# tqch/v-diffusion-torch

Measured on AMD Instinct MI355X. Metric: train_images_per_sec, higher is better.
Workload: dtype fp32 (bf16x3 split products in the tile-engine GEMMs)

## Files before the change

include/vdiff_hip.h:

```cpp
#ifndef VDIFF_HIP_H
#define VDIFF_HIP_H
#include <stddef.h>
#include <stdint.h>

#ifdef __cplusplus
extern "C" {
#endif

#define VD_VERSION 100

int         vd_version(void);
const char* vd_last_error(void);

int         vd_set_reserved_cus(int32_t n);
int         vd_reserved_cus(void);

int         vd_mfma_calibrate(float* sink, unsigned long long* stamps, int32_t blocks, int32_t iters, uint32_t seed, void* stream);

enum { VD_ROW = 0,
       VD_COL = 1,
       VD_IM2COL = 2 };

typedef struct vd_gemm_desc {
    const float* A; const float* B; float* C;
// ... 34 lines not shown
int vd_conv3x3_wino_supported(int32_t nimg, int32_t H, int32_t W, int32_t Cin, int32_t Cout, int64_t ldx, int64_t ldy, int64_t ldres);
int vd_conv3x3_wino(const float* xin, int64_t ldx, const float* U, const float* bias, const float* res, int64_t ldres,
                    float* y, int64_t ldy, int32_t nimg, int32_t H, int32_t W, int32_t Cin, int32_t Cout,
                    float* stats_part, void* stream);
int vd_conv3x3_wgrad_wino_supported(int32_t nimg, int32_t H, int32_t W, int32_t Cin, int32_t Cout, int64_t ldx, int64_t lddy);
size_t vd_conv3x3_wgrad_wino_ws_bytes(int32_t nimg, int32_t H, int32_t W, int32_t Cin, int32_t Cout);
int vd_conv3x3_wgrad_wino(const float* xin, int64_t ldx, const float* dy, int64_t lddy, int32_t nimg, int32_t H, int32_t W,
                          int32_t Cin, int32_t Cout, float* dw_oihw, float* dbias, int32_t Cin_w, int32_t Cout_w,
                          int32_t accumulate, float* ws, size_t ws_bytes, void* stream);
int vd_conv3x3_wgrad_wino_phase(const float* xin, int64_t ldx, const float* dy, int64_t lddy, int32_t nimg, int32_t H, int32_t W,
                                int32_t Cin, int32_t Cout, float* dw_oihw, float* dbias, int32_t Cin_w, int32_t Cout_w,
                                int32_t accumulate, float* ws, size_t ws_bytes, int32_t phase, void* stream);
int vd_wino_last_kernel(void);
int vd_wino_wgrad_last_kernel(void);
#ifdef VD_PROBES
int vd_wino_set_probe(unsigned long long* buf);
int vd_wino43_set_probe(unsigned long long* buf);
int vd_gn_set_spin_probe(unsigned* buf);
#endif
int vd_wino_pack(const float* w_oihw, int32_t Cout, int32_t Cin, float* uf , float* ud , void* stream);
int vd_conv3x3_dgrad_wino43_supported(int32_t nimg, int32_t H, int32_t W, int32_t Cin, int32_t Cout, int64_t lddy, int64_t lddx);
size_t vd_wino43_u_floats(int32_t Cout, int32_t Cin);
int vd_conv3x3_dgrad_wino43(const float* dy, int64_t lddy, const float* U43, float* dx, int64_t lddx, int32_t nimg, int32_t H, int32_t W,
                            int32_t Cin, int32_t Cout, void* stream);
int vd_wino43_last_kernel(void);
int vd_wino43_pack(const float* w_oihw, int32_t Cout, int32_t Cin, float* U43, void* stream);
int vd_wino43_pack_batched(const int64_t* items_dev, int32_t n, int64_t total_blocks, void* stream);
int vd_conv3x3_wino43_preferred(int32_t nimg, int32_t H, int32_t W, int32_t N);
int vd_conv3x3_wino43_fwd_supported(int32_t nimg, int32_t H, int32_t W, int32_t Cin, int32_t Cout, int64_t ldx, int64_t ldy, int64_t ldres);
int vd_wino43_pack_fwd(const float* w_oihw, int32_t Cout, int32_t Cin, float* U43f, void* stream);
int vd_conv3x3_wino43_fwd_chunk_rows(int32_t H, int32_t W);
int vd_conv3x3_wino43_fwd(const float* xin, int64_t ldx, const float* U43f, const float* bias, const float* res, int64_t ldres, float* y,
                          int64_t ldy, int32_t nimg, int32_t H, int32_t W, int32_t Cin, int32_t Cout, float* stats_part, void* stream);
int vd_conv3x3_wgrad_wino43_supported(int32_t nimg, int32_t H, int32_t W, int32_t Cin, int32_t Cout, int64_t ldx, int64_t lddy);
size_t vd_conv3x3_wgrad_wino43_ws_bytes(int32_t nimg, int32_t H, int32_t W, int32_t Cin, int32_t Cout);
int vd_conv3x3_wgrad_wino43(const float* xin, int64_t ldx, const float* dy, int64_t lddy, int32_t nimg, int32_t H, int32_t W,
                            int32_t Cin, int32_t Cout, float* dw_oihw, float* dbias, int32_t Cin_w, int32_t Cout_w,
                            int32_t accumulate, float* ws, size_t ws_bytes, void* stream);
int vd_conv3x3_wgrad_wino43_phase(const float* xin, int64_t ldx, const float* dy, int64_t lddy, int32_t nimg, int32_t H, int32_t W,
                                  int32_t Cin, int32_t Cout, float* dw_oihw, float* dbias, int32_t Cin_w, int32_t Cout_w,
                                  int32_t accumulate, float* ws, size_t ws_bytes, int32_t phase, void* stream);
int vd_wino43_wgrad_last_kernel(void);

int vd_wino_pack_batched(const int64_t* items_dev, int32_t n, int64_t total_blocks, void* stream);

int vd_im2col3x3(const float* x, int64_t ldx, float* xc , int32_t nimg, int32_t H, int32_t W, int32_t C, void* stream);
int vd_tap_gather(const float* z, int64_t ldz, const float* bias, float* out, int64_t ldo, int32_t nimg, int32_t H, int32_t W, int32_t Cout, void* stream);
int vd_tap_spread(const float* dy, int64_t lddy, float* dz, int64_t ldz, int32_t nimg, int32_t H, int32_t W, int32_t Cout, void* stream);
int vd_thin_wgrad_finish(const float* g, int32_t Cout_w, int32_t Cin, int32_t Cin_w, float* dw_oihw, int32_t accumulate,
                         const float* colsum, int32_t cs_stride, int32_t cs_off, float* dbias, void* stream);

size_t vd_conv3x3_wgrad_ws_bytes(int32_t nimg, int32_t H, int32_t W, int32_t Cin, int32_t Cout);
int vd_conv3x3_wgrad(const float* xin, int64_t ldx, const float* dy, int64_t lddy,
                     int32_t nimg, int32_t H, int32_t W, int32_t Cin, int32_t Cout,
                     float* dw_oihw, float* dbias, int32_t Cin_w, int32_t Cout_w, int32_t accumulate,
                     float* ws, size_t ws_bytes, void* stream);
int vd_conv3x3_wgrad_phase(const float* xin, int64_t ldx, const float* dy, int64_t lddy,
                           int32_t nimg, int32_t H, int32_t W, int32_t Cin, int32_t Cout,
                           float* dw_oihw, float* dbias, int32_t Cin_w, int32_t Cout_w, int32_t accumulate,
                           float* ws, size_t ws_bytes, int32_t phase, void* stream);

int vd_pack_conv3x3(const float* w_oihw, int32_t Cout_w, int32_t Cin_w,
                    float* wf, int32_t Cin_p, float* wd, int32_t Cout_p, void* stream);
int vd_pack_conv3x3_batched(const int64_t* items_dev, int32_t n, int64_t total_blocks, void* stream);

enum { VD_RS_NONE = 0, VD_RS_DOWN = 1, VD_RS_UP = 2 };

size_t vd_gn_ws_bytes(int32_t nimg, int32_t HW, int32_t C);
int vd_gn_stats(const float* x, int64_t ldx, int32_t nimg, int32_t HW, int32_t C, int32_t G, float eps,
                float* stats, float* ws, size_t ws_bytes, void* stream);

int vd_gn_stats_from_partials(const float* part1, int32_t C1, int32_t chunks1, const float* part2, int32_t C2, int32_t chunks2,
                              int32_t nimg, int32_t HW, int32_t G, float eps, float* stats, void* stream);

int vd_gn_coef_from_partials(const float* part1, int32_t C1, int32_t chunks1, const float* part2, int32_t C2, int32_t chunks2,
                             int32_t nimg, int32_t HW, int32_t G, float eps, const float* gamma, const float* beta,
                             const float* film, float* coef, void* stream);

int vd_gn_apply(const float* x, int64_t ldx, const float* stats, const float* gamma, const float* beta,
                const float* film, int32_t act, float p_drop, uint64_t seed,
                int32_t resample, float* y, int64_t ldy,
                int32_t nimg, int32_t H, int32_t W, int32_t C, int32_t G, float* coef, void* stream);

int vd_gn_apply_from_partials(const float* x, int64_t ldx, const float* part1, int32_t C1, int32_t chunks1, const float* part2, int32_t C2,
                              int32_t chunks2, const float* gamma, const float* beta, const float* film, int32_t act, float p_drop,
                              uint64_t seed, int32_t resample, float* y, int64_t ldy, int32_t nimg, int32_t H, int32_t W, int32_t C,
                              int32_t G, float eps, float* coef, void* stream);

int vd_gn_apply_bwd(const float* dy, int64_t lddy, const float* x, int64_t ldx, const float* coef,
                    const float* gamma, const float* beta, const float* film, int32_t act, float p_drop, uint64_t seed,
                    int32_t resample, const float* add, int64_t ldadd, float* dx, int64_t lddx, int32_t accumulate_dx,
                    float* dfilm, float* dgamma, float* dbeta, int32_t accumulate_params,
                    int32_t nimg, int32_t H, int32_t W, int32_t C, int32_t G,
                    float* ws, size_t ws_bytes, void* stream);
int vd_gn_bwd_last_kernel(void);
int vd_gn_apply_bwd_keep(const float* dy, int64_t lddy, const float* x, int64_t ldx, const float* coef, const float* gamma,
                         const float* beta, const float* film, int32_t act, float p_drop, uint64_t seed, int32_t resample,
                         const float* add, int64_t ldadd, float* dx, int64_t lddx, int32_t accumulate_dx, float* dfilm, float* pgb_keep,
                         int32_t nimg, int32_t H, int32_t W, int32_t C, int32_t G, float* ws, size_t ws_bytes, void* stream);
int vd_gn_param_sums_batched(const int64_t* items_dev, int32_t n, int64_t total_blocks, void* stream);

size_t vd_colsum_ws_bytes(int64_t M, int32_t N);
int vd_colsum(const float* x, int64_t ldx, int64_t M, int32_t N, float* out, int32_t accumulate,
              float* ws, size_t ws_bytes, void* stream);
int vd_axpby(const float* x, int64_t ldx, float alpha, float* y, int64_t ldy, float beta, int64_t rows, int32_t C, void* stream);
int vd_silu(const float* x, float* y, int64_t n, void* stream);
int vd_silu_bwd(const float* x, const float* dy, float* dx, int64_t n, int32_t accumulate, void* stream);
int vd_softmax_rows(float* s, int64_t rows, int32_t L, void* stream);
int vd_softmax_rows_bwd(const float* p, float* dp, int64_t rows, int32_t L, float alpha, void* stream);

int vd_attn_supported(int32_t L, int32_t hd, int32_t backward);
int vd_attn_fwd(const float* q, const float* k, const float* v, int64_t ld, float* o, int64_t ldo, float* lse, int32_t B,
                int32_t nh, int32_t L, int32_t hd, float scale, void* stream);
int vd_attn_bwd(const float* q, const float* k, const float* v, int64_t ld, const float* o, int64_t ldo, const float* dout,
                int64_t lddo, const float* lse, float* delta, float* dq, float* dk, float* dv, int64_t ldd, int32_t B,
                int32_t nh, int32_t L, int32_t hd, float scale, void* stream);
int vd_attn_bwd_phase(const float* q, const float* k, const float* v, int64_t ld, const float* o, int64_t ldo, const float* dout,
                      int64_t lddo, const float* lse, float* delta, float* dq, float* dk, float* dv, int64_t ldd, int32_t B,
                      int32_t nh, int32_t L, int32_t hd, float scale, int32_t phase, void* stream);

int vd_nchw_to_nhwc(const float* x, float* y, int32_t nimg, int32_t C, int32_t H, int32_t W, int64_t ldy, void* stream);
// ... 55 lines not shown
```

v-diffusion-torch_amd/csrc/common.h:

```cpp
#pragma once
#include <hip/hip_runtime.h>
#include <stdint.h>
#include <stdio.h>
#include "../../include/vdiff_hip.h"

typedef float f32x4 __attribute__((ext_vector_type(4)));
typedef float f32x16 __attribute__((ext_vector_type(16)));

typedef float f32x2 __attribute__((ext_vector_type(2)));

#ifdef VD_PROBES
constexpr bool VD_PROBE_BUILD = true;
#else
constexpr bool VD_PROBE_BUILD = false;
#endif

void vd_set_error(const char* fmt, ...);
int vd_cu_count(void);
int vd_persistent_cus(void);
int vd_gemm_grouped_wgrad_kblk(const float* const* A, const float* const* B, float* const* C, float* const* colsum, int32_t count, int32_t M,
                               int32_t N, int32_t K, int64_t lda, int64_t ldb, int64_t ldc, int32_t splitk, float* ws, size_t ws_bytes,
                               void* stream, int64_t a_kblk, int64_t b_kblk, int32_t slabs_only);
int vd_gemm_grouped_wgrad_used_slabs(int32_t count, int32_t M, int32_t N, int32_t K, int32_t splitk);
extern thread_local int vd_g_last_tile;
inline int vd_tile_code(bool tr, bool spl, int kt, int bm, int bn) {
    return ((((tr ? 1 : 0) + (spl ? 2 : 0)) * 100 + kt) * 1000 + bm) * 1000 + bn;
}

#define VD_REQUIRE(cond, ...)                                   \
    do { if (!(cond)) { vd_set_error(__VA_ARGS__); return 1; } } while (0)

#define VD_LAUNCH_CHECK(name)                                                            \
    do { hipError_t e_ = hipGetLastError();                                              \
         if (e_ != hipSuccess) { vd_set_error("%s: %s", name, hipGetErrorString(e_)); return 2; } } while (0)

static inline bool vd_aligned16(const void* p) { return (reinterpret_cast<uintptr_t>(p) & 15) == 0; }

__device__ __forceinline__ float vd_sigmoid(float x) { return __builtin_amdgcn_rcpf(1.0f + __expf(-x)); }

__device__ __forceinline__ void vd_philox4(uint64_t seed, uint64_t ctr, uint32_t out[4]) {
    uint32_t k0 = (uint32_t)seed, k1 = (uint32_t)(seed >> 32);
    uint32_t c0 = (uint32_t)ctr, c1 = (uint32_t)(ctr >> 32), c2 = 0x243F6A88u, c3 = 0x85A308D3u;
#pragma unroll
    for (int r = 0; r < 10; ++r) {
        uint64_t p0 = (uint64_t)0xD2511F53u * c0, p1 = (uint64_t)0xCD9E8D57u * c2;
        uint32_t n0 = (uint32_t)(p1 >> 32) ^ c1 ^ k0, n2 = (uint32_t)(p0 >> 32) ^ c3 ^ k1;
        c1 = (uint32_t)p1; c3 = (uint32_t)p0; c0 = n0; c2 = n2;
        k0 += 0x9E3779B9u; k1 += 0xBB67AE85u;
    }
    out[0] = c0; out[1] = c1; out[2] = c2; out[3] = c3;
}
__device__ __forceinline__ f32x4 vd_dropout_scale4(uint64_t seed, uint64_t vec_index, float p) {
    uint32_t r[4];
    vd_philox4(seed, vec_index, r);
    const float inv = 1.0f / (1.0f - p);
    f32x4 m;
#pragma unroll
    for (int j = 0; j < 4; ++j) m[j] = ((r[j] >> 8) * (1.0f / 16777216.0f) >= p) ? inv : 0.0f;
    return m;
}
```

v-diffusion-torch_amd/csrc/gemm.hip:

```cpp
#include "common.h"
#include <math.h>
#include <stdlib.h>
#include <type_traits>

namespace {

constexpr int KT = 32;
#ifndef VD_GEMM_SPLIT_DEFAULT
#define VD_GEMM_SPLIT_DEFAULT 1
#endif

struct GemmArgs {
    const float* A; const float* B; float* C; const float* bias; const float* R;
    int M, N, K;
    long long lda, ldb, ldc, ldr;
    int nh;
    long long sAb, sAh, sBb, sBh, sCb, sCh, sRb, sRh;
    float alpha; int accumulate;
    int H, W, Cin;
    int kt_total, kt_per_split;
    long long slab_stride;
    float* colsum; int colsum_accumulate;
    int probe;
    float* stats; int stats_hw;
    long long sBias;
    int group_S;
    int lgW, lgHW;
    long long a_kblk, b_kblk;
};

__device__ __forceinline__ int PB(const GemmArgs& p) { return VD_PROBE_BUILD ? p.probe : 0; }

__device__ __forceinline__ int row_swz(int row, int chunk) { return row * KT + ((chunk ^ ((row >> 1) & 7)) << 2); }

template <int BM, int BN, int AK, int BK, bool SPLITK>
__global__ __launch_bounds__(256, 2) void gemm_kernel(const GemmArgs p) {
    __shared__ __attribute__((aligned(16))) float smem[2 * (BM + BN) * KT];
    float* As = smem;
    float* Bs = smem + 2 * BM * KT;

    constexpr int MT = BM / 64, NT = BN / 64;
    constexpr int AIT = BM / 32, BIT = BN / 32;
    constexpr int A_CPR = BM / 4, A_RPP = 256 / A_CPR;
    constexpr int B_CPR = BN / 4, B_RPP = 256 / B_CPR;

    const int tid = threadIdx.x, lane = tid & 63, wave = tid >> 6;
    const int li = lane & 31, lh = lane >> 5;
    const int wm = (wave >> 1) * (BM / 2), wn = (wave & 1) * (BN / 2);
    const int m0 = blockIdx.y * BM;
    int n0 = blockIdx.x * BN;
    int tapN = 0, ci0 = 0;
    if (BK == VD_IM2COL) {
        const int cchN = (p.Cin + BN - 1) / BN;
        tapN = blockIdx.x / cchN;
        ci0 = (blockIdx.x % cchN) * BN;
        n0 = tapN * p.Cin + ci0;
    }
    const float* A = p.A;
    const float* B = p.B;
    float* C = p.C;
    const float* R = p.R;
// ... 378 lines not shown
            const int rowoff = (GROUPED && p.a_kblk) ? (kk >> 4) * (int)p.a_kblk + (kk & 15) * (int)p.lda : kk * (int)p.lda;
            voA[j] = (m0 + cm < p.M) ? (unsigned)(rowoff + cm) * 4u : OOB;
            kcA[j] = kk; mkA[j] = 0;
        } else {
            const int row = q * RRPP + lane / RLPR;
            const int c = (lane % RLPR) ^ swz_of<KT>(row);
            const int m = m0 + row;
            kcA[j] = c * 4;
            voA[j] = (m < p.M) ? (unsigned)(row * (int)p.lda + c * 4) * 4u : OOB;
            unsigned mk = 0;
            if (AK == VD_IM2COL) {
                int y, x;
                pix_yx(p, m, y, x);
                const unsigned xm = (x > 0 ? 1u : 0u) | 2u | (x < p.W - 1 ? 4u : 0u);
                mk = (y > 0 ? xm : 0u) | (xm << 3) | (y < p.H - 1 ? xm << 6 : 0u);
            }
            mkA[j] = mk;
        }
    }
#pragma unroll
    for (int j = 0; j < BIT; ++j) {
        const int q = j * 4 + wave;
        if (BK == VD_ROW) {
            const int row = q * RRPP + lane / RLPR;
            const int c = (lane % RLPR) ^ swz_of<KT>(row);
            kcB[j] = c * 4;
            voB[j] = (n0 + row < p.N) ? (unsigned)(row * (int)p.ldb + c * 4) * 4u : OOB;
            by[j] = bx[j] = 0;
        } else {
            const int kk = q * B_RPP + lane / B_LPR, cn = (lane % B_LPR) * 4;
            kcB[j] = kk;
            const bool ok = (BK == VD_IM2COL) ? (ci0 + cn < p.Cin) : (n0 + cn < p.N);
            const int rowoff = (GROUPED && BK == VD_COL && p.b_kblk) ? (kk >> 4) * (int)p.b_kblk + (kk & 15) * (int)p.ldb : kk * (int)p.ldb;
            voB[j] = ok ? (unsigned)(rowoff + cn) * 4u : OOB;
            if (BK == VD_IM2COL) pix_yx(p, kt_begin * KT + kk, by[j], bx[j]);
            else by[j] = bx[j] = 0;
        }
    }
    const float* Ablk = (AK == VD_COL) ? A + m0 : A + (long long)m0 * p.lda;
    const float* Bblk = (BK == VD_ROW) ? B + (long long)n0 * p.ldb : ((BK == VD_COL) ? B + n0 : B + ci0);
    const long long tapoffB = (BK == VD_IM2COL) ? (long long)((tapN / 3 - 1) * p.W + (tapN % 3 - 1)) * p.ldb : 0;

#ifndef VD_ISSUE_IN
#define VD_ISSUE_IN 2
#endif
    constexpr bool ISSUE_IN = VD_ISSUE_IN == 2 ? (AK == VD_COL) : (VD_ISSUE_IN == 1);
    struct Prep { const float* pA; const float* pB; unsigned vA[AIT], vB[BIT]; };
    auto prep_tiles = [&](int kt, Prep& P) {
        {
            const int tap = tapA, c0 = ccA * KT;
            long long aoff;
            int kwidth;
            if (AK == VD_IM2COL) { aoff = (long long)((tap / 3 - 1) * p.W + (tap % 3 - 1)) * p.lda + c0; kwidth = p.Cin - c0; }
            else if (AK == VD_ROW) { aoff = (long long)kt * KT; kwidth = p.K - kt * KT; }
            else { aoff = (GROUPED && p.a_kblk) ? (long long)kt * (KT / 16) * p.a_kblk : (long long)kt * KT * p.lda; kwidth = p.K - kt * KT; }
            P.pA = Ablk + aoff;
#pragma unroll
            for (int j = 0; j < AIT; ++j) {
                unsigned vo = voA[j];
                if (kcA[j] >= kwidth) vo = OOB;
                if (AK == VD_IM2COL && !((mkA[j] >> tap) & 1u)) vo = OOB;
                P.vA[j] = vo;
            }
        }
        {
            long long boff;
            int kwidth;
            if (BK == VD_ROW) {
                if (AK == VD_IM2COL) { boff = (long long)tapA * p.Cin + ccA * KT; kwidth = p.Cin - ccA * KT; }
                else { boff = (long long)kt * KT; kwidth = p.K - kt * KT; }
            } else { boff = ((GROUPED && BK == VD_COL && p.b_kblk) ? (long long)kt * (KT / 16) * p.b_kblk : (long long)kt * KT * p.ldb) + tapoffB; kwidth = p.K - kt * KT; }
            P.pB = Bblk + boff;
            const int dy = tapN / 3 - 1, dx = tapN % 3 - 1;
// ... 399 lines not shown
            if (lh == 0 && mrow < p.M) {
                const int chunks = p.stats_hw / (BM / 2);
                float* o = p.stats + ((long long)(mrow / p.stats_hw) * chunks + (mrow % p.stats_hw) / (BM / 2)) * 2 * p.N + n;
                o[0] = st1; o[p.N] = st2;
            }
        }
    }
    stamp_end();
}

template <int BM, int BN, int AK, int BK, bool SPLITK, int KT, bool TR, bool GROUPED = false>
__global__ __launch_bounds__(256, (KT == 16 ? VD_KT16_BLOCKS : 2)) void gemm_dma_kernel(const GemmArgs p,
                                                                                          const std::conditional_t<GROUPED, GroupPtrs, NoGroup> gp) {
    gemm_dma_body<BM, BN, AK, BK, SPLITK, KT, TR, GROUPED, false>(p, gp);
}
template <int BM, int BN, int AK, int BK, bool SPLITK, int KT, bool TR, bool GROUPED = false>
__global__ __launch_bounds__(256, (KT == 16 ? VD_SPL_BLOCKS : 2)) void gemm_split_kernel(const GemmArgs p,
                                                                                           const std::conditional_t<GROUPED, GroupPtrs, NoGroup> gp) {
    gemm_dma_body<BM, BN, AK, BK, SPLITK, KT, TR, GROUPED, true>(p, gp);
}

__global__ __launch_bounds__(512) void wgrad_planes256_kernel(const GemmArgs p, const GroupPtrs gp) {
    constexpr int BM = 256, BN = 256, KTT = 16, NBUF = 3, STG = (BM + BN) * KTT;
    __shared__ __attribute__((aligned(1024))) float smem[NBUF * STG];
    typedef float f32x2 __attribute__((ext_vector_type(2)));
    const int tid = threadIdx.x, lane = tid & 63;
    const int wave = __builtin_amdgcn_readfirstlane(tid >> 6);
    const int li = lane & 31, lh = lane >> 5;
    const int wm = (wave >> 1) * 64, wn = (wave & 1) * 128;
    const int tbx = blockIdx.x, tby = blockIdx.y, tbz = blockIdx.z;
    const int m0 = tby * BM, n0 = tbx * BN;
    const int e = tbz / p.group_S, slab = tbz - e * p.group_S;
    const float* A = gp.A[e] + m0;
    const float* B = gp.B[e] + n0;
    const int kt_begin = slab * p.kt_per_split, kt_end = min(kt_begin + p.kt_per_split, p.kt_total);
    float* C = p.C + (long long)tbz * p.slab_stride;

    auto issue = [&](int kt, int buf) {
        float* as = smem + buf * STG;
        float* bs = as + BM * KTT;
        const int rec = kt < kt_end ? (int)OOB : 0;
        const __amdgpu_buffer_rsrc_t rsA = make_rsrc(A + (p.a_kblk ? (long long)kt * p.a_kblk : (long long)kt * KTT * p.lda), rec);
        const __amdgpu_buffer_rsrc_t rsB = make_rsrc(B + (p.b_kblk ? (long long)kt * p.b_kblk : (long long)kt * KTT * p.ldb), rec);
#pragma unroll
        for (int h = 0; h < 2; ++h) {
            const int kk = wave + 8 * h;
            __builtin_amdgcn_raw_ptr_buffer_load_lds(rsA, (lds_ptr_t)(as + kk * BM), 16, lane * 16, kk * (int)p.lda * 4, 0, 0);
            __builtin_amdgcn_raw_ptr_buffer_load_lds(rsB, (lds_ptr_t)(bs + kk * BN), 16, lane * 16, kk * (int)p.ldb * 4, 0, 0);
        }
    };

    f32x16 acc[2][4];
#pragma unroll
    for (int a = 0; a < 2; ++a)
#pragma unroll
        for (int b = 0; b < 4; ++b)
#pragma unroll
            for (int r = 0; r < 16; ++r) acc[a][b][r] = 0.f;
    float csum[2] = {0.f, 0.f};
    const bool do_cs = p.colsum != nullptr && tbx == 0 && (wave & 1) == 0;

    if (kt_begin < kt_end) {
        issue(kt_begin, 0);
        issue(kt_begin + 1, 1);
        asm volatile("s_waitcnt vmcnt(4)" ::: "memory");
        asm volatile("s_waitcnt lgkmcnt(0)\n\ts_barrier" ::: "memory");
        int buf = 0;
        for (int kt = kt_begin; kt < kt_end; ++kt) {
            const float* as = smem + buf * STG;
            const float* bs = as + BM * KTT;
            issue(kt + 2, buf >= 1 ? buf - 1 : 2);
            float fa[2][8];
            f32x4 fbq[8];
#pragma unroll
            for (int j = 0; j < 8; ++j) {
                const f32x2 v = *reinterpret_cast<const f32x2*>(as + (8 * lh + j) * BM + wm + 2 * li);
                fa[0][j] = v[0]; fa[1][j] = v[1];
                fbq[j] = *reinterpret_cast<const f32x4*>(bs + (8 * lh + j) * BN + wn + 4 * li);
            }
            bf16x8 ah[2], am[2], al[2];
#pragma unroll
// ... 400 lines not shown
    return g;
}
}

extern "C" int vd_gemm_grouped_wgrad_auto_split(int32_t count, int32_t M, int32_t N, int32_t K, int32_t min_slabs, int32_t max_slabs) {
    const int tile = choose_tile(M, N, false, (long long)count * 8, 0);
    const bool p256 = planes256(count, M, N, K);
    long long nm, nn;
    grouped_tiles(tile, p256, M, N, &nm, &nn);
    const long long blocks = nm * nn * count;
    const long long slots = (long long)vd_cu_count() * (p256 ? 1 : (tile == 0 && blocks * (min_slabs > 1 ? min_slabs : 1) >= GROUPED_K16_MIN_WGS / 2 ? 4 : TILES[tile].per_cu));
    int lo = min_slabs > 1 ? min_slabs : 1, hi = max_slabs > lo ? max_slabs : lo;
    const int kmax = K / 256 > 1 ? K / 256 : 1;
    if (hi > kmax) hi = kmax;
    if (lo > hi) lo = hi;
    int best = lo;
    double best_eff = -1.0;
    for (int s = lo; s <= hi; ++s) {
        const long long wgs = blocks * s, rounds = (wgs + slots - 1) / slots;
        double eff = (double)wgs / (double)(rounds * slots);
        eff *= 1.0 - 0.004 * s;
        if (eff > best_eff) { best_eff = eff; best = s; }
    }
    return best;
}

extern "C" size_t vd_gemm_grouped_wgrad_ws_bytes(int32_t count, int32_t M, int32_t N, int32_t splitk) {
    return (size_t)count * (splitk > 1 ? splitk : 1) * ((size_t)M * N + M) * sizeof(float);
}

extern "C" int vd_gemm_grouped_wgrad(const float* const* A, const float* const* B, float* const* C, float* const* colsum, int32_t count,
                                     int32_t M, int32_t N, int32_t K, int64_t lda, int64_t ldb, int64_t ldc, int32_t splitk, float* ws,
                                     size_t ws_bytes, void* stream) {
    return vd_gemm_grouped_wgrad_kblk(A, B, C, colsum, count, M, N, K, lda, ldb, ldc, splitk, ws, ws_bytes, stream, 0, 0, 0);
}

int vd_gemm_grouped_wgrad_used_slabs(int32_t count, int32_t M, int32_t N, int32_t K, int32_t splitk) {
    return plan_grouped(count, M, N, K, splitk > 1 ? splitk : 1).used;
}

int vd_gemm_grouped_wgrad_kblk(const float* const* A, const float* const* B, float* const* C, float* const* colsum, int32_t count,
                               int32_t M, int32_t N, int32_t K, int64_t lda, int64_t ldb, int64_t ldc, int32_t splitk, float* ws,
                               size_t ws_bytes, void* stream, int64_t a_kblk, int64_t b_kblk, int32_t slabs_only) {
    VD_REQUIRE(A && B && C && count > 0 && count <= VD_GROUP_MAX, "vd_gemm_grouped_wgrad: 1..%d entries (got %d)", VD_GROUP_MAX, count);
    VD_REQUIRE(M > 0 && N > 0 && K > 0 && M % 4 == 0 && N % 4 == 0 && lda % 4 == 0 && ldb % 4 == 0 && ldc >= N,
               "vd_gemm_grouped_wgrad: M, N, lda, ldb must be multiples of 4 (M=%d N=%d)", M, N);
    const int S = splitk > 1 ? splitk : 1;
    VD_REQUIRE(ws && ws_bytes >= vd_gemm_grouped_wgrad_ws_bytes(count, M, N, S), "vd_gemm_grouped_wgrad: workspace too small");
    GemmArgs a = {};
    GroupPtrs gp = {};
    GroupOut go = {};
    for (int e = 0; e < count; ++e) {
        VD_REQUIRE(A[e] && B[e] && C[e] && vd_aligned16(A[e]) && vd_aligned16(B[e]), "vd_gemm_grouped_wgrad: entry %d: null / unaligned operand", e);
        gp.A[e] = A[e]; gp.B[e] = B[e]; go.C[e] = C[e]; go.cs[e] = colsum ? colsum[e] : nullptr;
    }
    a.A = A[0]; a.B = B[0];
    a.M = M; a.N = N; a.K = K; a.lda = lda; a.ldb = ldb; a.ldc = N; a.ldr = 0; a.nh = 1;
    a.alpha = 1.f; a.lgW = a.lgHW = -1; a.probe = 0;
    a.a_kblk = a_kblk; a.b_kblk = b_kblk;
    VD_REQUIRE(a_kblk >= 0 && b_kblk >= 0 && a_kblk % 4 == 0 && b_kblk % 4 == 0 && 2 * a_kblk + 16 * lda + 128 < 0x70000000LL / 4 &&
               2 * b_kblk + 16 * ldb + 128 < 0x70000000LL / 4, "vd_gemm_grouped_wgrad: K-block strides outside the LDS-DMA kernel's range");
    VD_REQUIRE(dma_in_range(a), "vd_gemm_grouped_wgrad: operands outside the LDS-DMA kernel's range (alignment / row pitch)");
    const GroupedPlan g = plan_grouped(count, M, N, K, S);
    const int used = g.used;
    a.kt_total = g.kt_total; a.kt_per_split = g.kt_per_split; a.group_S = used;
    a.slab_stride = (long long)M * N;
    a.C = ws;
    float* cpart = ws + (long long)count * used * a.slab_stride;
    a.colsum = colsum ? cpart : nullptr;
    const dim3 grid((unsigned)g.nn, (unsigned)g.nm, (unsigned)(count * used));
    hipStream_t st = (hipStream_t)stream;
    if (g.p256) {
        vd_g_last_tile = vd_tile_code(true, true, 16, 256, 256);
        hipLaunchKernelGGL(wgrad_planes256_kernel, grid, dim3(512), 0, st, a, gp);
    } else if (g.tile == 0 && g.k16) launch_grouped<128, 128, 16>(a, gp, grid, st);
    else if (g.tile == 0) launch_grouped<128, 128>(a, gp, grid, st);
    else if (g.tile == 1) launch_grouped<128, 64>(a, gp, grid, st);
    else if (g.tile == 2) launch_grouped<64, 128>(a, gp, grid, st);
    else launch_grouped<64, 64>(a, gp, grid, st);
    VD_LAUNCH_CHECK("gemm_dma_kernel(grouped)");
    if (slabs_only) return 0;
    const long long tot = (long long)M * N;
    hipLaunchKernelGGL(reduce_slabs_grouped_kernel, dim3((unsigned)((tot + 255) / 256), (unsigned)count), dim3(256), 0, st, ws, used,
                       a.slab_stride, M, N, go, (long long)ldc, cpart);
    VD_LAUNCH_CHECK("reduce_slabs_grouped_kernel");
    return 0;
}

thread_local int vd_g_last_tile = 0;
extern "C" int vd_gemm_last_tile(void) { return vd_g_last_tile; }

extern "C" int vd_gemm(const vd_gemm_desc* d, void* stream) {
// ... 127 lines not shown
```

v-diffusion-torch_amd/csrc/norm.hip:

```cpp
#include "common.h"
#include <stdlib.h>

namespace {

constexpr int PPC = 128;

template <bool NT>
__device__ __forceinline__ f32x4 ld_stream(const float* p) {
    if (NT) return __builtin_nontemporal_load(reinterpret_cast<const f32x4*>(p));
    return *reinterpret_cast<const f32x4*>(p);
}
template <bool NT>
__device__ __forceinline__ void st_stream(float* p, f32x4 v) {
    if (NT) __builtin_nontemporal_store(v, reinterpret_cast<f32x4*>(p));
    else *reinterpret_cast<f32x4*>(p) = v;
}

struct ReduceArgs {
    const float* x; long long ldx;
    const float* dy; long long lddy;
    const float* coef;
    int act; float p_drop; unsigned long long seed; int resample; int has_norm;
    int H, W;
    long long HW;
// ... 279 lines not shown
    const float* ximg = p.x + (long long)b * p.H * p.W * p.ldx;
    float* yimg = p.y + (long long)b * Ho * Wo * p.ldy;
    if (p.resample == VD_RS_NONE) {
        for (int i = r; i < np; i += 4 * rows) {
            f32x4 v[4];
#pragma unroll
            for (int u = 0; u < 4; ++u)
                if (i + u * rows < np) v[u] = *reinterpret_cast<const f32x4*>(ximg + (long long)(p0 + i + u * rows) * p.ldx + c4);
#pragma unroll
            for (int u = 0; u < 4; ++u)
                if (i + u * rows < np) {
                    const int po = p0 + i + u * rows;
                    *reinterpret_cast<f32x4*>(yimg + (long long)po * p.ldy + c4) = fwd_val(p, v[u], po, c4, sc, of, b);
                }
        }
        return;
    }
    for (int i = r; i < np; i += rows) {
        const int po = p0 + i;
        f32x4 out;
        {
            const int yo = po / Wo, xo = po - yo * Wo;
            if (p.resample == VD_RS_UP) out = fwd_one(p, ximg, (yo >> 1) * p.W + (xo >> 1), c4, sc, of, b);
            else {
                const int q = (2 * yo) * p.W + 2 * xo;
                out = (fwd_one(p, ximg, q, c4, sc, of, b) + fwd_one(p, ximg, q + 1, c4, sc, of, b) +
                       fwd_one(p, ximg, q + p.W, c4, sc, of, b) + fwd_one(p, ximg, q + p.W + 1, c4, sc, of, b)) * 0.25f;
            }
        }
        *reinterpret_cast<f32x4*>(yimg + (long long)po * p.ldy + c4) = out;
    }
}

__global__ __launch_bounds__(256) void gn_bwd_finalize_kernel(const float* part, int chunks, const float* coef,
                                                              const float* gamma, const float* beta, const float* film,
                                                              int C, int G, long long HW, float* q, float* dfilm,
                                                              float* pgb) {
    extern __shared__ float sh[];
    float* k1 = sh; float* k2 = sh + C; float* gm = sh + 2 * C;
    const int b = blockIdx.x, cg = C / G;
    const float* cf = coef + (long long)b * 4 * C;
    for (int c = threadIdx.x; c < C; c += blockDim.x) {
        float s1 = 0.f, s2 = 0.f;
        for (int ch = 0; ch < chunks; ++ch) {
            const float* pp = part + ((long long)(b * chunks + ch) * 2) * C;
            s1 += pp[c]; s2 += pp[C + c];
        }
        float fs = 1.f;
        if (film) {
            fs = 1.f + film[(long long)b * 2 * C + C + c];
            dfilm[(long long)b * 2 * C + c] = s1;
            dfilm[(long long)b * 2 * C + C + c] = gamma[c] * s2 + beta[c] * s1;
        }
        const float k = gamma[c] * fs;
        k1[c] = k * s1; k2[c] = k * s2;
        pgb[((long long)b * 2) * C + c] = fs * s2;
        pgb[((long long)b * 2 + 1) * C + c] = fs * s1;
    }
    __syncthreads();
    if (threadIdx.x < G) {
        float m1 = 0.f, m2 = 0.f;
        for (int c = threadIdx.x * cg; c < (threadIdx.x + 1) * cg; ++c) { m1 += k1[c]; m2 += k2[c]; }
        const float inv = 1.f / ((float)cg * (float)HW);
        gm[threadIdx.x] = m1 * inv; gm[G + threadIdx.x] = m2 * inv;
    }
    __syncthreads();
// ... 442 lines not shown
    const long long Wo = resample == VD_RS_DOWN ? W / 2 : (resample == VD_RS_UP ? W * 2 : W);
    const int Cba = pick_cb(C);
    VD_REQUIRE(C % Cba == 0 && Cba % 4 == 0 && Cba <= 1024 && nimg <= 65535, "vd_gn_apply: cannot split C=%d / nimg=%d", C, nimg);
    hipLaunchKernelGGL(gn_apply_kernel<false>, dim3((unsigned)((Ho * Wo + APIX - 1) / APIX), nimg, C / Cba), dim3(256), 0, st, p, Cba, PartArgs{});
    VD_LAUNCH_CHECK("gn_apply_kernel");
    return 0;
}

extern "C" int vd_gn_apply_from_partials(const float* x, int64_t ldx, const float* part1, int32_t C1, int32_t chunks1, const float* part2,
                                         int32_t C2, int32_t chunks2, const float* gamma, const float* beta, const float* film, int32_t act,
                                         float p_drop, uint64_t seed, int32_t resample, float* y, int64_t ldy, int32_t nimg, int32_t H,
                                         int32_t W, int32_t C, int32_t G, float eps, float* coef, void* stream) {
    hipStream_t st = (hipStream_t)stream;
    VD_REQUIRE(x && y && part1 && gamma && beta, "vd_gn_apply_from_partials: null operand");
    VD_REQUIRE(C % 4 == 0 && ldx % 4 == 0 && ldy % 4 == 0 && C % G == 0 && C1 + C2 == C && C1 > 0 && chunks1 > 0,
               "vd_gn_apply_from_partials: bad channel split C=%d C1=%d C2=%d G=%d", C, C1, C2, G);
    VD_REQUIRE(C2 == 0 || (part2 && chunks2 > 0), "vd_gn_apply_from_partials: second source incomplete");
    VD_REQUIRE(resample != VD_RS_DOWN || (H % 2 == 0 && W % 2 == 0), "vd_gn_apply_from_partials: odd size cannot be average-pooled");
    VD_REQUIRE(vd_aligned16(x) && vd_aligned16(y) && (!coef || vd_aligned16(coef)), "vd_gn_apply_from_partials: operands must be 16-byte aligned");
    ApplyArgs p = {x, ldx, coef, 1, act, p_drop, seed, resample, y, ldy, nimg, H, W, C};
    PartArgs q = {part1, C1, chunks1, part2, C2, chunks2, G, eps, gamma, beta, film, coef};
    const long long Ho = resample == VD_RS_DOWN ? H / 2 : (resample == VD_RS_UP ? H * 2 : H);
    const long long Wo = resample == VD_RS_DOWN ? W / 2 : (resample == VD_RS_UP ? W * 2 : W);
    const int cg = C / G;
    int Cba = pick_cb(C);
    if (Cba % cg) {
        Cba = 0;
        for (int k = G; k >= 1; --k) if (G % k == 0 && (k * cg) % 4 == 0 && k * cg <= 1024) { Cba = k * cg; break; }
    }
    VD_REQUIRE(Cba > 0 && C % Cba == 0 && Cba % 4 == 0 && Cba % cg == 0 && Cba <= 1024 && Cba / cg <= 256 && nimg <= 65535,
               "vd_gn_apply_from_partials: cannot split C=%d into whole-group channel ranges", C);
    hipLaunchKernelGGL(gn_apply_kernel<true>, dim3((unsigned)((Ho * Wo + APIX - 1) / APIX), nimg, C / Cba), dim3(256), 0, st, p, Cba, q);
    VD_LAUNCH_CHECK("gn_apply_kernel<from partials>");
    return 0;
}

static int gn_apply_bwd_impl(const float* dy, int64_t lddy, const float* x, int64_t ldx, const float* coef,
                             const float* gamma, const float* beta, const float* film, int32_t act, float p_drop,
                             uint64_t seed, int32_t resample, const float* add, int64_t ldadd, float* dx, int64_t lddx,
                             int32_t accumulate_dx, float* dfilm, float* dgamma, float* dbeta, int32_t accumulate_params,
                             int32_t nimg, int32_t H, int32_t W, int32_t C, int32_t G, float* ws, size_t ws_bytes,
                             float* pgb_keep, void* stream) {
    hipStream_t st = (hipStream_t)stream;
    VD_REQUIRE(C % 4 == 0 && lddy % 4 == 0 && lddx % 4 == 0, "vd_gn_apply_bwd: C/ld must be multiples of 4");
    const int has_norm = gamma != nullptr;
    const long long HW = (long long)H * W;
    BwdApplyArgs a = {};
    ReduceArgs& p = a.r;
    p.x = x; p.ldx = ldx; p.dy = dy; p.lddy = lddy; p.coef = coef; p.act = act; p.p_drop = p_drop; p.seed = seed;
    p.resample = resample; p.has_norm = has_norm; p.H = H; p.W = W; p.HW = HW; p.C = C; p.nimg = nimg;
    p.chunks = (int)((HW + PPC - 1) / PPC);
    a.add = add; a.ldadd = ldadd; a.dx = dx; a.lddx = lddx; a.accumulate_dx = accumulate_dx;
    g_last_gn_bwd = has_norm ? -1 : 0;
    if (has_norm) {
        VD_REQUIRE(x && coef && beta && ((dgamma && dbeta) || pgb_keep) && C % G == 0 && ldx % 4 == 0, "vd_gn_apply_bwd: missing norm operands");
        VD_REQUIRE(!film || dfilm, "vd_gn_apply_bwd: film given without dfilm");
        VD_REQUIRE(ws && ws_bytes >= vd_gn_ws_bytes(nimg, (int)HW, C), "vd_gn_apply_bwd: workspace too small");
        const int Cb = pick_cb(C);
        VD_REQUIRE(C % Cb == 0 && Cb % 4 == 0 && Cb <= 1024, "vd_gn_apply_bwd: cannot split C=%d", C);
        float* part = ws;
        float* q = part + (long long)nimg * p.chunks * 2 * C;
        float* pgb = pgb_keep ? pgb_keep : q + (long long)nimg * 3 * C;
        p.part = part;
        static const bool two_pass = getenv("VD_GN_TWO_PASS") != nullptr;
        int CS = fused_slab(C, G);
        static const bool wide = !(getenv("VD_GN_WIDE") && atoi(getenv("VD_GN_WIDE")) == 0);
// ... 125 lines not shown
```

v-diffusion-torch_amd/csrc/wino43.hip:

```cpp
#include "common.h"
#include <type_traits>

namespace {

typedef __attribute__((address_space(3))) void* lds_ptr_t;
constexpr unsigned OOB = 0x80000000u;
constexpr int KT = 8;
constexpr int TN = 32;
constexpr int TILES = 64;
constexpr int U_STAGE = 36 * 4 * 16 * 2 * 2;
constexpr int THREADS = 512;

struct Args43 {
    const float* x; long long ldx;
    const float* U;
    float* y; long long ldy;
    int nimg, H, W, K, N;
    int items_per_img;
    int ngrp;
    int ncb, nitems;
    const float* bias; const float* res; long long ldr;
    float* stats;
    int chunks_per_img;
    unsigned long long* probe;
// ... 29 lines not shown
    } else {
        const T c = d[4] - d[2], e = d[3] - d[1];
        o0 = c + 2.f * e;
        o1 = c - 2.f * e;
        o2 = 4.f * d[1] + (d[5] - 5.f * d[3]);
    }
}
template <bool DY, typename T>
__device__ __forceinline__ void bt_full(const T (&r)[6], T (&v)[6]) {
    if (DY) {
        const T e1 = r[4] - 2.25f * r[2], f1 = r[3] - 2.25f * r[1];
        const T e2 = r[4] - 0.5625f * r[2], f2 = r[3] - 0.5625f * r[1];
        v[0] = 1.265625f * r[0] + (r[4] - 2.8125f * r[2]);
        v[1] = e1 + 0.75f * f1;
        v[2] = e1 - 0.75f * f1;
        v[3] = e2 + 1.5f * f2;
        v[4] = e2 - 1.5f * f2;
        v[5] = 1.265625f * r[1] + (r[5] - 2.8125f * r[3]);
        return;
    }
    const T t = r[4] - 4.f * r[2], u = r[3] - 4.f * r[1], c = r[4] - r[2], e = r[3] - r[1];
    v[0] = 4.f * r[0] + (r[4] - 5.f * r[2]);
    v[1] = t + u;
    v[2] = t - u;
    v[3] = c + 2.f * e;
    v[4] = c - 2.f * e;
    v[5] = 4.f * r[1] + (r[5] - 5.f * r[3]);
}
template <int HALF, bool DY>
__device__ __forceinline__ void bt_half2(const f32x2 (&d)[6], f32x2& o0, f32x2& o1, f32x2& o2) { bt_half<HALF, DY, f32x2>(d, o0, o1, o2); }
template <bool DY>
__device__ __forceinline__ void bt_full2(const f32x2 (&r)[6], f32x2 (&v)[6]) { bt_full<DY, f32x2>(r, v); }

template <int TWT, bool FWD>
__global__ __launch_bounds__(THREADS) void wino43_conv_kernel(const Args43 p) {
    constexpr bool QUAD = TWT == 4;
    constexpr int RUN = TWT + 1;
    constexpr int RUNS = QUAD ? 4 * RUN - 2 : 4 * RUN;
    constexpr int RP = QUAD ? RUNS + 1 : RUNS + ((TWT / 4) & 3);
    constexpr int NTR = TILES / TWT;
    constexpr int RIN = QUAD ? 4 * 17 + 1 : 4 * NTR + 2;
    constexpr int NS = RIN * RP;
    constexpr int NPG = (NS + 63) / 64;
    constexpr int A_STAGE = 2 * NPG * 256;
    constexpr int STAGE = A_STAGE + U_STAGE;
    constexpr int LGT = TWT == 4 ? 2 : TWT == 8 ? 3 : 4;
    static_assert((4 * RP * 16) % 256 == (TWT * 16) % 256 || (QUAD && (4 * RP * 16) % 256 == 192), "row pitch leaves bank conflicts");
    static_assert(2 * STAGE * 4 <= 163840, "stages exceed the LDS");
    static_assert(8 * 16 * 64 * 16 + 8 * 4 * 8 * 4 <= 2 * STAGE * 4, "epilogue exchange + statistics area exceeds the stages");
    __shared__ __attribute__((aligned(1024))) float smem[2 * STAGE];

    const int tid = threadIdx.x, lane = tid & 63;
    const int wave = __builtin_amdgcn_readfirstlane(tid >> 6);
    const int li = lane & 15, lq = lane >> 4;
    const int tg = wave & 3;
    const int nkt = p.K / KT;
    const int G = gridDim.x;
    int probe_n = 0;
    auto stamp = [&](int slot) {
        if (VD_PROBE_BUILD && p.probe && probe_n < 4) {
            const unsigned long long t = slot == 12 ? __builtin_amdgcn_s_memrealtime() : __builtin_amdgcn_s_memtime();
            if (lane == 0) p.probe[(((long long)blockIdx.x * 8 + wave) * 4 + probe_n) * 16 + slot] = t;
        }
    };
    auto stamp_val = [&](int slot, unsigned long long v) {
        if (VD_PROBE_BUILD && p.probe && probe_n < 4 && lane == 0) p.probe[(((long long)blockIdx.x * 8 + wave) * 4 + probe_n) * 16 + slot] = v;
    };

// ... 9 lines not shown
            const int s = (wave >> 1) + 4 * j;
            const int slot = s * 64 + lane;
            const int r = slot / RP, cs = slot - r * RP;
            int c, idx, yy, im;
            if (QUAD) {
                c = cs >= 3 * RUN - 1 ? 3 : cs >= 2 * RUN ? 2 : cs >= RUN ? 1 : 0;
                idx = cs - (c * RUN - (c == 3 ? 1 : 0));
                const int i4 = r / 17;
                im = i4; yy = r - 17 * i4 - 1;
                if (i4 >= 4) yy = -1;
            } else {
                c = cs / RUN; idx = cs - c * RUN;
                im = 0; yy = y_first + r;
            }
            const int xx = 4 * idx + c - 1;
            unsigned vo = OOB;
            if (s < NPG && r < RIN && cs < RUNS && (unsigned)xx < (unsigned)p.W && (unsigned)yy < (unsigned)p.H)
                vo = (unsigned)(((im * p.H + yy) * p.W + xx) * (int)p.ldx) * 4u;
            pxo[j] = vo;
        }
    };
    auto issue_piece = [&](int i, int kt, int st, int cb) {
        float* sb = smem + st * STAGE;
        if (i < 5) {
            const int q = wave + 8 * i;
            if (q < 36) {
                const float* src = p.U + ((long long)cb * nkt + kt) * U_STAGE;
                const __amdgpu_buffer_rsrc_t rs = make_rsrc(src);
                __builtin_amdgcn_raw_ptr_buffer_load_lds(rs, (lds_ptr_t)(sb + A_STAGE + q * 256), 16, lane * 16, q * 1024, 0, 0);
            }
        } else {
            const int j = i - 5;
            const int s = (wave >> 1) + 4 * j, g = wave & 1;
            if (s < NPG) {
                const __amdgpu_buffer_rsrc_t rs = make_rsrc(xitem + kt * KT);
                __builtin_amdgcn_raw_ptr_buffer_load_lds(rs, (lds_ptr_t)(sb + (g * NPG + s) * 256), 16, (int)pxo[j], g * 16, 0, 0);
            }
        }
    };
    constexpr int NPIECE = 5 + APL;
    constexpr int SB = SB_STEP, NAFTER = 18 - SB, PAFTER = NAFTER;
    constexpr int UPF = U_AHEAD;
    static_assert(PAFTER <= NPIECE && NPIECE - PAFTER <= SB, "DMA schedule does not fit the tile");

    const int tl = 16 * tg + li;
    const int tyl = tl >> LGT, tx = tl & (TWT - 1);
    const int prow0 = QUAD ? 17 * (tyl >> 2) + 4 * (tyl & 3) : 4 * tyl;
    const int pbase = ((lq >> 1) * NPG * 64 + prow0 * RP + tx) * 4 + (lq & 1) * 2;
    auto poff = [](int pr, int q) { return (pr * RP + ((q & 3) * RUN - (QUAD && (q & 3) == 3 ? 1 : 0)) + (q >> 2)) * 4; };
    const int uoff = A_STAGE + lane * 4;

    const int ngrp = p.ngrp;
    auto item_of = [&](int n, int& cb, int& grp) -> bool {
        int t = n * G + (int)blockIdx.x;
        if ((G & 7) == 0 && (n + 1) * G <= p.nitems) t = n * G + ((int)blockIdx.x & 7) * (G >> 3) + ((int)blockIdx.x >> 3);
        if (t >= p.nitems) return false;
        if ((p.ncb & 3) == 0 && (ngrp & 7) == 0) {
            const int c = t >> 5, i = t & 31, ncg = p.ncb >> 2;
            cb = (c % ncg) * 4 + (i & 3); grp = (c / ncg) * 8 + (i >> 2);
            return true;
        }
        cb = t % p.ncb; grp = t / p.ncb;
        return true;
    };

    auto run = [&](auto Hc) {
        constexpr int HALF = decltype(Hc)::value;
        auto rowpass = [&](const float* sa, f32x2 (&Rn)[3][6], int q0, int q1) {
#pragma unroll
            for (int q = 0; q < 6; ++q) {
                if (q < q0 || q >= q1) continue;
                f32x2 d[6];
#pragma unroll
                for (int pr = 0; pr < 6; ++pr) {
                    if ((HALF == 0 && pr == 5) || (HALF == 1 && pr == 0)) d[pr] = f32x2{0.f, 0.f};
                    else d[pr] = *(const volatile __attribute__((address_space(3))) f32x2*)((const __attribute__((address_space(3))) float*)sa + poff(pr, q));
                }
                bt_half2<HALF, FWD>(d, Rn[0][q], Rn[1][q], Rn[2][q]);
            }
        };
        auto first_stage = [&](int cbx, int grpx) {
            if (QUAD) xitem = p.x + (long long)grpx * (4 * 16 * 16) * p.ldx;
            else { offsets(grpx); xitem = p.x + (long long)(grpx / p.items_per_img) * p.H * p.W * p.ldx; }
#pragma unroll
            for (int i = 0; i < NPIECE; ++i) issue_piece(i, 0, 0, cbx);
        };
        int cb = 0, grp = 0, cb_next = 0, grp_next = 0;
        if (QUAD) offsets(0);
        bool have = item_of(0, cb, grp);
        if (have) first_stage(cb, grp);
        for (int n = 0; have; ++n) {
            probe_n = n;
            stamp(0); stamp(12);
            unsigned long long t_vm = 0, t_bar = 0;
            f32x4 acc[18][2];
#pragma unroll
            for (int x = 0; x < 18; ++x) { acc[x][0] = f32x4{0.f, 0.f, 0.f, 0.f}; acc[x][1] = f32x4{0.f, 0.f, 0.f, 0.f}; }
            if (n == 0) asm volatile("s_waitcnt vmcnt(0)" ::: "memory");
            else asm volatile("s_waitcnt vmcnt(16)" ::: "memory");
            lds_barrier();
            stamp(1);
            if (nkt > 1) {
#pragma unroll
                for (int i = 0; i < PAFTER; ++i) issue_piece(i, 1, 1, cb);
            }
            f32x2 R[3][6];
            rowpass(smem + pbase, R, 0, 6);
            stamp(2);
            for (int kt = 0; kt < nkt; ++kt) {
                const int st = kt & 1;
                const float* su = smem + st * STAGE + uoff;
                const float* san = smem + (st ^ 1) * STAGE + pbase;
                const bool n1 = kt + 1 < nkt, n2 = kt + 2 < nkt;
                f32x2 Rn[3][6];
                f32x4 uf[UPF + 1], ufl[NAFTER];
#pragma unroll
                for (int e = 0; e < UPF; ++e) uf[e] = *reinterpret_cast<const f32x4*>(su + (18 * HALF + e) * 256);
#pragma unroll
                for (int a = 0; a < 3; ++a) {
                    f32x2 V[6];
                    bt_full2<FWD>(R[a], V);
#pragma unroll
                    for (int b = 0; b < 6; ++b) {
                        const int xl = 6 * a + b;
                        if (xl == SB) {
#pragma unroll
                            for (int e = 0; e < NAFTER; ++e) ufl[e] = *reinterpret_cast<const f32x4*>(su + (18 * HALF + SB + e) * 256);
                            if (VD_PROBE_BUILD && p.probe) {
                                const unsigned long long ta = __builtin_amdgcn_s_memtime();
                                asm volatile("s_waitcnt vmcnt(0)" ::: "memory");
                                const unsigned long long tb = __builtin_amdgcn_s_memtime();
                                __syncthreads();
                                const unsigned long long tc = __builtin_amdgcn_s_memtime();
                                t_vm += tb - ta; t_bar += tc - tb;
                            } else {
                                asm volatile("s_waitcnt vmcnt(0)" ::: "memory");
                                __syncthreads();
                            }
                        }
                        if (xl + UPF < SB) uf[(xl + UPF) % (UPF + 1)] = *reinterpret_cast<const f32x4*>(su + (18 * HALF + xl + UPF) * 256);
                        if (xl + PAFTER < NPIECE) { if (n1) issue_piece(xl + PAFTER, kt + 1, st ^ 1, cb); }
                        if (xl >= SB) {
                            if (n2) issue_piece(xl - SB, kt + 2, st, cb);
                            rowpass(san, Rn, (6 * (xl - SB)) / NAFTER, (6 * (xl - SB + 1)) / NAFTER);
                        }
                        const f32x4 u = xl < SB ? uf[xl % (UPF + 1)] : ufl[xl < SB ? 0 : xl - SB];
                        acc[xl][0] = __builtin_amdgcn_mfma_f32_16x16x4f32(u[0], V[b][0], acc[xl][0], 0, 0, 0);
                        acc[xl][1] = __builtin_amdgcn_mfma_f32_16x16x4f32(u[2], V[b][0], acc[xl][1], 0, 0, 0);
                        acc[xl][0] = __builtin_amdgcn_mfma_f32_16x16x4f32(u[1], V[b][1], acc[xl][0], 0, 0, 0);
                        acc[xl][1] = __builtin_amdgcn_mfma_f32_16x16x4f32(u[3], V[b][1], acc[xl][1], 0, 0, 0);
                    }
                }
#pragma unroll
                for (int a = 0; a < 3; ++a)
#pragma unroll
                    for (int q = 0; q < 6; ++q) R[a][q] = Rn[a][q];
            }
            stamp(3);
            __syncthreads();
            stamp(4);

            f32x4* xch = reinterpret_cast<f32x4*>(smem);
            const int lane_e = FWD ? (int)__builtin_amdgcn_mbcnt_hi(~0u, __builtin_amdgcn_mbcnt_lo(~0u, 0u)) : lane;
            const int li_e = lane_e & 15, lq_e = lane_e >> 4;
            const int tl_e = 16 * tg + li_e, tyl_e = tl_e >> LGT, tx_e = tl_e & (TWT - 1);
            f32x4 Y[4][4];
            f32x4 RV[FWD ? 4 : 1][FWD ? 4 : 1];
#pragma unroll
            for (int pass = 0; pass < 2; ++pass) {
                const int blk = pass == 0 ? 1 - HALF : HALF;
                f32x4 S[3][4];
#pragma unroll
                for (int a = 0; a < 3; ++a) {
                    const f32x4 m0 = acc[6 * a][blk], m1 = acc[6 * a + 1][blk], m2 = acc[6 * a + 2][blk], m3 = acc[6 * a + 3][blk],
                                m4 = acc[6 * a + 4][blk], m5 = acc[6 * a + 5][blk];
                    const f32x4 p12 = m1 + m2, q12 = m1 - m2, p34 = m3 + m4, q34 = m3 - m4;
                    S[a][0] = m0 + p12 + p34;
                    if (FWD) {
                        S[a][1] = 0.75f * q12 + 1.5f * q34;
                        S[a][2] = 0.5625f * p12 + 2.25f * p34;
                        S[a][3] = 0.421875f * q12 + 3.375f * q34 + m5;
                    } else {
                        S[a][1] = q12 + 2.f * q34;
                        S[a][2] = p12 + 4.f * p34;
                        S[a][3] = q12 + 8.f * q34 + m5;
                    }
                }
#pragma unroll
                for (int v = 0; v < 4; ++v) {
// ... 137 lines not shown
    double Gm[6][3];
#pragma unroll
    for (int a = 0; a < 6; ++a)
#pragma unroll
        for (int c = 0; c < 3; ++c) Gm[a][c] = fwd ? Gd[a][c] : Gc[a][c];
    double tmp[6][3];
#pragma unroll
    for (int a = 0; a < 6; ++a)
#pragma unroll
        for (int c = 0; c < 3; ++c) tmp[a][c] = Gm[a][0] * g[0][c] + Gm[a][1] * g[1][c] + Gm[a][2] * g[2][c];
    float* dst = U + ((long long)nb * nkt + kt) * U_STAGE + t;
#pragma unroll
    for (int a = 0; a < 6; ++a)
#pragma unroll
        for (int b = 0; b < 6; ++b)
            dst[(6 * a + b) * 256] = (float)(tmp[a][0] * Gm[b][0] + tmp[a][1] * Gm[b][1] + tmp[a][2] * Gm[b][2]);
}

__global__ __launch_bounds__(256) void wino43_pack_kernel(const float* w, float* U, int Cout, int Cin, int fwd) {
    pack43_tile(w, U, Cout, Cin, blockIdx.x, fwd);
}

__global__ __launch_bounds__(256) void wino43_pack_batched_kernel(const long long* items, int n) {
    int lo = 0, hi = n - 1;
    while (lo < hi) {
        const int mid = (lo + hi + 1) >> 1;
        if (items[8 * mid + 7] <= (long long)blockIdx.x) lo = mid; else hi = mid - 1;
    }
    const long long* it = items + 8 * lo;
    pack43_tile(reinterpret_cast<const float*>(it[0]), reinterpret_cast<float*>(it[1]), (int)it[3], (int)it[4],
                (int)((long long)blockIdx.x - it[7]), (int)it[2]);
}

__device__ __forceinline__ void bt6(const f32x4 (&d)[6], f32x4 (&o)[6]) {
    const f32x4 e1 = d[4] - 2.25f * d[2], f1 = 0.75f * d[3] - 1.6875f * d[1];
    const f32x4 e2 = d[4] - 0.5625f * d[2], f2 = 1.5f * d[3] - 0.84375f * d[1];
    o[0] = 1.265625f * d[0] + (d[4] - 2.8125f * d[2]);
    o[1] = e1 + f1;
    o[2] = e1 - f1;
    o[3] = e2 + f2;
    o[4] = e2 - f2;
    o[5] = 1.265625f * d[1] + (d[5] - 2.8125f * d[3]);
}
__device__ __forceinline__ void a6(const f32x4 (&y)[4], f32x4 (&o)[6]) {
    const f32x4 e1 = y[0] + 0.5625f * y[2], f1 = 0.75f * y[1] + 0.421875f * y[3];
    const f32x4 e2 = y[0] + 2.25f * y[2], f2 = 1.5f * y[1] + 3.375f * y[3];
    o[0] = y[0];
    o[1] = e1 + f1;
    o[2] = e1 - f1;
    o[3] = e2 + f2;
    o[4] = e2 - f2;
    o[5] = y[3];
}

__device__ __forceinline__ void st_once(float* p, f32x4 v) { *reinterpret_cast<f32x4*>(p) = v; }
struct WgT43 {
    const float* x; long long ldx; const float* dy; long long lddy;
    float* V; float* dM;
    int nimg, H, W, Cin, Cout, TW, TPI, T;
};

__global__ __launch_bounds__(256) void wino43_wgrad_transform_kernel(const WgT43 p) {
    const int quad = blockIdx.y * 64 + threadIdx.x, tile = blockIdx.x * 4 + threadIdx.y;
    if (tile >= p.T) return;
    const int img = tile / p.TPI, tin = tile - img * p.TPI;
    const int ty = tin / p.TW, tx = tin - ty * p.TW;
    const int c4 = 4 * quad;
    if (blockIdx.z == 0) {
        if (c4 >= p.Cin) return;
        f32x4 R[6][6];
#pragma unroll
        for (int pr = 0; pr < 6; ++pr) {
            const int yy = 4 * ty - 1 + pr;
            f32x4 d[6];
#pragma unroll
            for (int q = 0; q < 6; ++q) {
                const int xx = 4 * tx - 1 + q;
                d[q] = f32x4{0.f, 0.f, 0.f, 0.f};
                if ((unsigned)yy < (unsigned)p.H && (unsigned)xx < (unsigned)p.W)
                    d[q] = *reinterpret_cast<const f32x4*>(p.x + ((long long)(img * p.H + yy) * p.W + xx) * p.ldx + c4);
            }
            bt6(d, R[pr]);
        }
#pragma unroll
        for (int b = 0; b < 6; ++b) {
            f32x4 col[6], o[6];
#pragma unroll
            for (int pr = 0; pr < 6; ++pr) col[pr] = R[pr][b];
            bt6(col, o);
#pragma unroll
            for (int a = 0; a < 6; ++a)
                st_once(p.V + ((long long)((tile >> 4) * 36 + 6 * a + b) * 16 + (tile & 15)) * p.Cin + c4, o[a]);
        }
    } else {
        if (c4 >= p.Cout) return;
        f32x4 R[4][6];
#pragma unroll
        for (int u = 0; u < 4; ++u) {
            f32x4 y[4];
#pragma unroll
            for (int v = 0; v < 4; ++v)
// ... 82 lines not shown
        float u[6] = {0.f, 0.f, 0.f, 0.f, 0.f, 0.f};
        if (in) {
            const float* sl = slabs + (long long)b * S * plane + idx;
            const long long astep = 6LL * S * plane;
            for (int z = 0; z < S; ++z) {
#pragma unroll
                for (int a = 0; a < 6; ++a) u[a] += sl[a * astep + z * plane];
            }
        }
        const float s12 = u[1] + u[2], d12 = u[2] - u[1], s34 = u[3] + u[4], d34 = u[3] - u[4];
        tsh[0][b][x] = g0 * u[0] - g12 * s12 + g34 * s34;
        tsh[1][b][x] = h12 * d12 + h34 * d34;
        tsh[2][b][x] = k * (s34 - s12) + u[5];
    }
    __syncthreads();
    if (!in || b >= 3) return;
    const int co = (int)(idx / Cin), ci = (int)(idx - (long long)co * Cin);
    if (co >= Cout_w || ci >= Cin_w) return;
    const int r = b;
    float t[6];
#pragma unroll
    for (int c = 0; c < 6; ++c) t[c] = tsh[r][c][x];
    const float s12 = t[1] + t[2], d12 = t[2] - t[1], s34 = t[3] + t[4], d34 = t[3] - t[4];
    const float w0 = g0 * t[0] - g12 * s12 + g34 * s34;
    const float w1 = h12 * d12 + h34 * d34;
    const float w2 = k * (s34 - s12) + t[5];
    float* o = dw + ((long long)co * Cin_w + ci) * 9 + 3 * r;
    o[0] = accumulate ? o[0] + w0 : w0;
    o[1] = accumulate ? o[1] + w1 : w1;
    o[2] = accumulate ? o[2] + w2 : w2;
}

struct Wg43Plan { bool ok; int T, S; size_t v_f, m_f, u_f, cs_f, gemm_bytes; };
Wg43Plan wg43_plan(int nimg, int H, int W, int Cin, int Cout) {
    Wg43Plan g = {};
    if (nimg <= 0 || H % 4 || W % 4 || H < 4 || W < 4 || Cin % 4 || Cout % 4) return g;
    g.T = nimg * (H / 4) * (W / 4);
    g.S = vd_gemm_grouped_wgrad_auto_split(36, Cout, Cin, g.T, (g.T + 1535) / 1536, 24);
    const size_t T16 = ((size_t)g.T + 15) / 16 * 16;
    g.v_f = (size_t)36 * T16 * Cin; g.m_f = (size_t)36 * T16 * Cout; g.u_f = (size_t)36 * Cout * Cin; g.cs_f = (size_t)36 * Cout;
    g.gemm_bytes = vd_gemm_grouped_wgrad_ws_bytes(36, Cout, Cin, g.S);
    g.ok = true;
    return g;
}

thread_local int g_last43 = 0;
#ifdef VD_PROBES
unsigned long long* g_probe43 = nullptr;
#else
constexpr unsigned long long* g_probe43 = nullptr;
#endif
thread_local int g_last43w = 0;

}

extern "C" int vd_conv3x3_dgrad_wino43_supported(int32_t nimg, int32_t H, int32_t W, int32_t Cin, int32_t Cout, int64_t lddy, int64_t lddx) {
    if (nimg <= 0 || Cout % KT || Cin % TN || lddy % 4 || lddx % 4) return 0;
    if (!((W == 32 && H == 32) || (W == 64 && H % 16 == 0 && H >= 16) || (W == 16 && H == 16 && nimg % 4 == 0))) return 0;
    const long long px = (W == 16 ? (long long)nimg : 1LL) * H * W, lim = 0x7FFFFFF0LL / 4;
    if (px * lddy >= lim || px * lddx >= lim) return 0;
    return 1;
}

extern "C" size_t vd_wino43_u_floats(int32_t Cout, int32_t Cin) { return (size_t)36 * Cout * Cin; }

extern "C" int vd_conv3x3_wino43_preferred(int32_t nimg, int32_t H, int32_t W, int32_t N) {
    if (nimg <= 0 || N <= 0) return 0;
    const long long grp = W == 16 ? (nimg + 3) / 4 : (long long)nimg * (W == 64 ? H / 16 : 1);
    const long long i43 = grp * ((N + TN - 1) / TN), ncu = vd_persistent_cus();
    const long long r43 = (i43 + ncu - 1) / ncu, r23 = (4 * i43 + ncu - 1) / ncu;
    return 8 * r43 < 3 * r23;
}

// ... 56 lines not shown

extern "C" int vd_conv3x3_wino43_fwd(const float* xin, int64_t ldx, const float* U43f, const float* bias, const float* res, int64_t ldres,
                                     float* y, int64_t ldy, int32_t nimg, int32_t H, int32_t W, int32_t Cin, int32_t Cout,
                                     float* stats_part, void* stream) {
    VD_REQUIRE(xin && U43f && y, "vd_conv3x3_wino43_fwd: null operand");
    VD_REQUIRE(vd_conv3x3_wino43_fwd_supported(nimg, H, W, Cin, Cout, ldx, ldy, res ? ldres : 0),
               "vd_conv3x3_wino43_fwd: unsupported geometry nimg=%d H=%d W=%d Cin=%d Cout=%d", nimg, H, W, Cin, Cout);
    VD_REQUIRE(vd_aligned16(xin) && vd_aligned16(U43f) && vd_aligned16(y) && (!res || vd_aligned16(res)) && (!bias || vd_aligned16(bias)),
               "vd_conv3x3_wino43_fwd: operands must be 16-byte aligned");
    Args43 a = {};
    a.x = xin; a.ldx = ldx; a.U = U43f; a.y = y; a.ldy = ldy;
    a.nimg = nimg; a.H = H; a.W = W; a.K = Cin; a.N = Cout;
    a.items_per_img = W == 64 ? H / 16 : 1;
    a.ngrp = W == 16 ? nimg / 4 : nimg * a.items_per_img;
    a.ncb = Cout / TN;
    a.bias = bias; a.res = res; a.ldr = ldres; a.stats = stats_part;
    a.chunks_per_img = (H * W) / vd_conv3x3_wino43_fwd_chunk_rows(H, W);
    VD_REQUIRE(a.chunks_per_img == a.items_per_img, "vd_conv3x3_wino43_fwd: statistics chunks (%d per image) do not match the work items (%d)", a.chunks_per_img, a.items_per_img);
    const long long items = (long long)a.ngrp * a.ncb;
    VD_REQUIRE(items < (1LL << 30), "vd_conv3x3_wino43_fwd: too many work items");
    a.nitems = (int)items;
    a.probe = g_probe43;
    const int ncu = vd_persistent_cus();
    const dim3 grid((unsigned)(items < ncu ? items : ncu)), blk(THREADS);
    hipStream_t st = (hipStream_t)stream;
    if (W == 16) hipLaunchKernelGGL((wino43_conv_kernel<4, true>), grid, blk, 0, st, a);
    else if (W == 32) hipLaunchKernelGGL((wino43_conv_kernel<8, true>), grid, blk, 0, st, a);
    else hipLaunchKernelGGL((wino43_conv_kernel<16, true>), grid, blk, 0, st, a);
    VD_LAUNCH_CHECK("wino43_conv_kernel<., true>");
    g_last43 = -(W / 4);
    return 0;
}

extern "C" int vd_wino43_pack_batched(const int64_t* items_dev, int32_t n, int64_t total_blocks, void* stream) {
    VD_REQUIRE(items_dev && n > 0 && total_blocks > 0 && total_blocks < (1LL << 31), "vd_wino43_pack_batched: bad table");
    hipLaunchKernelGGL(wino43_pack_batched_kernel, dim3((unsigned)total_blocks), dim3(256), 0, (hipStream_t)stream,
                       reinterpret_cast<const long long*>(items_dev), n);
    VD_LAUNCH_CHECK("wino43_pack_batched_kernel");
    return 0;
}

extern "C" int vd_conv3x3_wgrad_wino43_supported(int32_t nimg, int32_t H, int32_t W, int32_t Cin, int32_t Cout, int64_t ldx, int64_t lddy) {
    const Wg43Plan g = wg43_plan(nimg, H, W, Cin, Cout);
    if (!g.ok || ldx % 4 || lddy % 4 || g.T < 512 || g.T % 4) return 0;
    const long long px = (long long)nimg * H * W, lim = 0x7FFFFFF0LL / 4;
    if (px * ldx >= lim || px * lddy >= lim) return 0;
    if ((long long)g.T * (Cin > Cout ? Cin : Cout) * 4 >= (1LL << 40)) return 0;
    return 1;
}

extern "C" size_t vd_conv3x3_wgrad_wino43_ws_bytes(int32_t nimg, int32_t H, int32_t W, int32_t Cin, int32_t Cout) {
    const Wg43Plan g = wg43_plan(nimg, H, W, Cin, Cout);
    if (!g.ok) return 0;
    return (g.v_f + g.m_f + g.u_f + g.cs_f) * sizeof(float) + g.gemm_bytes;
}

static int wgrad43_impl(const float* xin, int64_t ldx, const float* dy, int64_t lddy, int32_t nimg, int32_t H, int32_t W, int32_t Cin,
                        int32_t Cout, float* dw_oihw, float* dbias, int32_t Cin_w, int32_t Cout_w, int32_t accumulate, float* ws,
                        size_t ws_bytes, void* stream, int phases) {
    VD_REQUIRE(xin && dy && dw_oihw && ws, "vd_conv3x3_wgrad_wino43: null operand");
    VD_REQUIRE(vd_conv3x3_wgrad_wino43_supported(nimg, H, W, Cin, Cout, ldx, lddy),
               "vd_conv3x3_wgrad_wino43: unsupported geometry nimg=%d H=%d W=%d Cin=%d Cout=%d", nimg, H, W, Cin, Cout);
    VD_REQUIRE(Cin_w <= Cin && Cout_w <= Cout, "vd_conv3x3_wgrad_wino43: real dims exceed padded dims");
    VD_REQUIRE(vd_aligned16(xin) && vd_aligned16(dy) && vd_aligned16(ws), "vd_conv3x3_wgrad_wino43: operands must be 16-byte aligned");
    VD_REQUIRE(ws_bytes >= vd_conv3x3_wgrad_wino43_ws_bytes(nimg, H, W, Cin, Cout), "vd_conv3x3_wgrad_wino43: workspace too small");
    const Wg43Plan g = wg43_plan(nimg, H, W, Cin, Cout);
    float* V = ws;
    float* dM = V + g.v_f;
    float* dU = dM + g.m_f;
    float* cs = dU + g.u_f;
    float* gws = cs + g.cs_f;
    hipStream_t st = (hipStream_t)stream;
    if (phases & 1) {
        WgT43 t = {};
        t.x = xin; t.ldx = ldx; t.dy = dy; t.lddy = lddy; t.V = V; t.dM = dM;
        t.nimg = nimg; t.H = H; t.W = W; t.Cin = Cin; t.Cout = Cout; t.TW = W / 4; t.TPI = (H / 4) * (W / 4); t.T = g.T;
        const int cmax = Cin > Cout ? Cin : Cout;
        hipLaunchKernelGGL(wino43_wgrad_transform_kernel, dim3((unsigned)(g.T / 4), (unsigned)((cmax + 255) / 256), 2), dim3(64, 4), 0, st, t);
        VD_LAUNCH_CHECK("wino43_wgrad_transform_kernel");
    }
    if (phases & 2) {
        const float* A[36]; const float* B[36]; float* C[36]; float* colsum[36];
        for (int e = 0; e < 36; ++e) {
            A[e] = dM + (size_t)e * 16 * Cout; B[e] = V + (size_t)e * 16 * Cin;
            C[e] = dU + (size_t)e * Cout * Cin; colsum[e] = cs + (size_t)e * Cout;
        }
        const int rc = vd_gemm_grouped_wgrad_kblk(A, B, C, colsum, 36, Cout, Cin, g.T, Cout, Cin, Cin, g.S, gws, g.gemm_bytes, stream,
                                                  36LL * 16 * Cout, 36LL * 16 * Cin,
                                                  (long long)Cout * Cin >= FUSED_FINISH_MIN ? 1 : 0);
        if (rc) return rc;
        g_last43w = g.S;
    }
    if (phases & 4) {
        const long long tot = (long long)Cout * Cin;
        if (tot >= FUSED_FINISH_MIN) {
            const int used = vd_gemm_grouped_wgrad_used_slabs(36, Cout, Cin, g.T, g.S);
            hipLaunchKernelGGL(wino43_wgrad_reduce_finish_kernel, dim3((unsigned)((tot + 63) / 64)), dim3(64, 6), 0, st, gws,
                               gws + (size_t)36 * used * Cout * Cin, used, Cout, Cin, Cout_w, Cin_w, dw_oihw, dbias, accumulate);
        } else {
            hipLaunchKernelGGL(wino43_wgrad_finish_kernel, dim3((unsigned)((tot + 255) / 256)), dim3(256), 0, st, dU, cs, Cout, Cin, Cout_w, Cin_w,
                               dw_oihw, dbias, accumulate);
        }
        VD_LAUNCH_CHECK("wino43_wgrad_finish_kernel");
    }
    return 0;
}

extern "C" int vd_conv3x3_wgrad_wino43(const float* xin, int64_t ldx, const float* dy, int64_t lddy, int32_t nimg, int32_t H, int32_t W,
                                       int32_t Cin, int32_t Cout, float* dw_oihw, float* dbias, int32_t Cin_w, int32_t Cout_w,
                                       int32_t accumulate, float* ws, size_t ws_bytes, void* stream) {
    return wgrad43_impl(xin, ldx, dy, lddy, nimg, H, W, Cin, Cout, dw_oihw, dbias, Cin_w, Cout_w, accumulate, ws, ws_bytes, stream, 7);
}

extern "C" int vd_conv3x3_wgrad_wino43_phase(const float* xin, int64_t ldx, const float* dy, int64_t lddy, int32_t nimg, int32_t H,
                                             int32_t W, int32_t Cin, int32_t Cout, float* dw_oihw, float* dbias, int32_t Cin_w,
                                             int32_t Cout_w, int32_t accumulate, float* ws, size_t ws_bytes, int32_t phase, void* stream) {
    VD_REQUIRE(phase == 1 || phase == 2 || phase == 4, "vd_conv3x3_wgrad_wino43_phase: phase must be 1 (transforms), 2 (GEMMs) or 4 (reduction + finish)");
    return wgrad43_impl(xin, ldx, dy, lddy, nimg, H, W, Cin, Cout, dw_oihw, dbias, Cin_w, Cout_w, accumulate, ws, ws_bytes, stream, phase);
}

extern "C" int vd_wino43_wgrad_last_kernel(void) { return g_last43w; }
```

v-diffusion-torch_amd/v_diffusion/_hip.py:

```python
import ctypes as C
import os

import torch

_HERE = os.path.dirname(os.path.abspath(__file__))
LIB_PATH = os.environ.get("VDIFF_HIP_LIB") or os.path.join(os.path.dirname(_HERE), "lib", "libvdiff_hip.so")

ROW, COL, IM2COL = 0, 1, 2
RS_NONE, RS_DOWN, RS_UP = 0, 1, 2
OUT_TYPES = {"v": 0, "x0": 1, "eps": 2, "both": 3}
REWEIGHTS = {"constant": 0, "snr": 1, "snr_trunc": 2, "snr_1plus": 3}

_i32, _i64, _f32, _f64, _u64, _vp, _sz = C.c_int32, C.c_int64, C.c_float, C.c_double, C.c_uint64, C.c_void_p, C.c_size_t


class GemmDesc(C.Structure):
    _fields_ = [("A", _vp), ("B", _vp), ("C", _vp), ("bias", _vp), ("R", _vp),
                ("M", _i32), ("N", _i32), ("K", _i32), ("a_kind", _i32), ("b_kind", _i32),
                ("lda", _i64), ("ldb", _i64), ("ldc", _i64), ("ldr", _i64),
                ("batch", _i32), ("nh", _i32),
                ("sAb", _i64), ("sAh", _i64), ("sBb", _i64), ("sBh", _i64),
                ("sCb", _i64), ("sCh", _i64), ("sRb", _i64), ("sRh", _i64),
                ("alpha", _f32), ("accumulate", _i32), ("H", _i32), ("W", _i32), ("Cin", _i32),
                ("splitk", _i32), ("ws", _vp), ("ws_bytes", _i64), ("tile", _i32),
# ... 2 lines not shown

_SIGNATURES = {
    "vd_version": (C.c_int, []),
    "vd_last_error": (C.c_char_p, []),
    "vd_set_reserved_cus": (C.c_int, [_i32]),
    "vd_reserved_cus": (C.c_int, []),
    "vd_mfma_calibrate": (C.c_int, [_vp, _vp, _i32, _i32, C.c_uint32, _vp]),
    "vd_gemm": (C.c_int, [C.POINTER(GemmDesc), _vp]),
    "vd_gemm_last_tile": (C.c_int, []),
    "vd_gemm_split_forms": (C.c_int, []),
    "vd_gemm_grouped_wgrad_ws_bytes": (_sz, [_i32, _i32, _i32, _i32]),
    "vd_gemm_grouped_wgrad_auto_split": (C.c_int, [_i32, _i32, _i32, _i32, _i32, _i32]),
    "vd_gemm_grouped_wgrad": (C.c_int, [_vp, _vp, _vp, _vp, _i32, _i32, _i32, _i32, _i64, _i64, _i64, _i32, _vp, _sz, _vp]),
    "vd_conv3x3": (C.c_int, [_vp, _i64, _vp, _vp, _vp, _i64, _vp, _i64, _i32, _i32, _i32, _i32, _i32, _i32, _vp, _vp]),
    "vd_conv3x3_wino_supported": (C.c_int, [_i32, _i32, _i32, _i32, _i32, _i64, _i64, _i64]),
    "vd_conv3x3_wino": (C.c_int, [_vp, _i64, _vp, _vp, _vp, _i64, _vp, _i64, _i32, _i32, _i32, _i32, _i32, _vp, _vp]),
    "vd_wino_pack": (C.c_int, [_vp, _i32, _i32, _vp, _vp, _vp]),
    "vd_conv3x3_wgrad_wino_supported": (C.c_int, [_i32, _i32, _i32, _i32, _i32, _i64, _i64]),
    "vd_conv3x3_wgrad_wino_ws_bytes": (_sz, [_i32, _i32, _i32, _i32, _i32]),
    "vd_conv3x3_wgrad_wino": (C.c_int, [_vp, _i64, _vp, _i64, _i32, _i32, _i32, _i32, _i32, _vp, _vp, _i32, _i32, _i32, _vp, _sz, _vp]),
    "vd_conv3x3_wgrad_wino_phase": (C.c_int, [_vp, _i64, _vp, _i64, _i32, _i32, _i32, _i32, _i32, _vp, _vp, _i32, _i32, _i32, _vp, _sz, _i32, _vp]),
    "vd_wino_last_kernel": (C.c_int, []),
    "vd_wino_wgrad_last_kernel": (C.c_int, []),
    "vd_wino_pack_batched": (C.c_int, [_vp, _i32, _i64, _vp]),
    "vd_conv3x3_dgrad_wino43_supported": (C.c_int, [_i32, _i32, _i32, _i32, _i32, _i64, _i64]),
    "vd_wino43_u_floats": (_sz, [_i32, _i32]),
    "vd_conv3x3_dgrad_wino43": (C.c_int, [_vp, _i64, _vp, _vp, _i64, _i32, _i32, _i32, _i32, _i32, _vp]),
    "vd_wino43_last_kernel": (C.c_int, []),
    "vd_conv3x3_wino43_fwd_supported": (C.c_int, [_i32, _i32, _i32, _i32, _i32, _i64, _i64, _i64]),
    "vd_conv3x3_wino43_preferred": (C.c_int, [_i32, _i32, _i32, _i32]),
    "vd_wino43_pack_fwd": (C.c_int, [_vp, _i32, _i32, _vp, _vp]),
    "vd_conv3x3_wino43_fwd_chunk_rows": (C.c_int, [_i32, _i32]),
    "vd_conv3x3_wino43_fwd": (C.c_int, [_vp, _i64, _vp, _vp, _vp, _i64, _vp, _i64, _i32, _i32, _i32, _i32, _i32, _vp, _vp]),
    "vd_wino43_pack": (C.c_int, [_vp, _i32, _i32, _vp, _vp]),
    "vd_wino43_pack_batched": (C.c_int, [_vp, _i32, _i64, _vp]),
    "vd_conv3x3_wgrad_wino43_supported": (C.c_int, [_i32, _i32, _i32, _i32, _i32, _i64, _i64]),
    "vd_conv3x3_wgrad_wino43_ws_bytes": (_sz, [_i32, _i32, _i32, _i32, _i32]),
    "vd_conv3x3_wgrad_wino43": (C.c_int, [_vp, _i64, _vp, _i64, _i32, _i32, _i32, _i32, _i32, _vp, _vp, _i32, _i32, _i32, _vp, _sz, _vp]),
    "vd_wino43_wgrad_last_kernel": (C.c_int, []),
    "vd_conv3x3_wgrad_wino43_phase": (C.c_int, [_vp, _i64, _vp, _i64, _i32, _i32, _i32, _i32, _i32, _vp, _vp, _i32, _i32, _i32, _vp, _sz, _i32, _vp]),
    "vd_gn_stats_from_partials": (C.c_int, [_vp, _i32, _i32, _vp, _i32, _i32, _i32, _i32, _i32, _f32, _vp, _vp]),
    "vd_gn_coef_from_partials": (C.c_int, [_vp, _i32, _i32, _vp, _i32, _i32, _i32, _i32, _i32, _f32, _vp, _vp, _vp, _vp, _vp]),
    "vd_conv3x3_wgrad_ws_bytes": (_sz, [_i32, _i32, _i32, _i32, _i32]),
    "vd_conv3x3_wgrad": (C.c_int, [_vp, _i64, _vp, _i64, _i32, _i32, _i32, _i32, _i32, _vp, _vp, _i32, _i32, _i32, _vp, _sz, _vp]),
    "vd_conv3x3_wgrad_phase": (C.c_int, [_vp, _i64, _vp, _i64, _i32, _i32, _i32, _i32, _i32, _vp, _vp, _i32, _i32, _i32, _vp, _sz, _i32, _vp]),
    "vd_pack_conv3x3": (C.c_int, [_vp, _i32, _i32, _vp, _i32, _vp, _i32, _vp]),
    "vd_pack_conv3x3_batched": (C.c_int, [_vp, _i32, _i64, _vp]),
    "vd_gn_ws_bytes": (_sz, [_i32, _i32, _i32]),
    "vd_gn_stats": (C.c_int, [_vp, _i64, _i32, _i32, _i32, _i32, _f32, _vp, _vp, _sz, _vp]),
    "vd_gn_apply": (C.c_int, [_vp, _i64, _vp, _vp, _vp, _vp, _i32, _f32, _u64, _i32, _vp, _i64, _i32, _i32, _i32, _i32, _i32, _vp, _vp]),
    "vd_gn_apply_from_partials": (C.c_int, [_vp, _i64, _vp, _i32, _i32, _vp, _i32, _i32, _vp, _vp, _vp, _i32, _f32, _u64, _i32, _vp, _i64, _i32,
                                            _i32, _i32, _i32, _i32, _f32, _vp, _vp]),
    "vd_gn_apply_bwd": (C.c_int, [_vp, _i64, _vp, _i64, _vp, _vp, _vp, _vp, _i32, _f32, _u64, _i32, _vp, _i64, _vp, _i64, _i32,
                                  _vp, _vp, _vp, _i32, _i32, _i32, _i32, _i32, _i32, _vp, _sz, _vp]),
    "vd_gn_bwd_last_kernel": (C.c_int, []),
    "vd_gn_apply_bwd_keep": (C.c_int, [_vp, _i64, _vp, _i64, _vp, _vp, _vp, _vp, _i32, _f32, _u64, _i32, _vp, _i64, _vp, _i64, _i32,
                                       _vp, _vp, _i32, _i32, _i32, _i32, _i32, _vp, _sz, _vp]),
    "vd_gn_param_sums_batched": (C.c_int, [_vp, _i32, _i64, _vp]),
    "vd_colsum_ws_bytes": (_sz, [_i64, _i32]),
    "vd_colsum": (C.c_int, [_vp, _i64, _i64, _i32, _vp, _i32, _vp, _sz, _vp]),
    "vd_axpby": (C.c_int, [_vp, _i64, _f32, _vp, _i64, _f32, _i64, _i32, _vp]),
    "vd_silu": (C.c_int, [_vp, _vp, _i64, _vp]),
    "vd_silu_bwd": (C.c_int, [_vp, _vp, _vp, _i64, _i32, _vp]),
    "vd_softmax_rows": (C.c_int, [_vp, _i64, _i32, _vp]),
    "vd_softmax_rows_bwd": (C.c_int, [_vp, _vp, _i64, _i32, _f32, _vp]),
    "vd_attn_supported": (C.c_int, [_i32, _i32, _i32]),
    "vd_attn_fwd": (C.c_int, [_vp, _vp, _vp, _i64, _vp, _i64, _vp, _i32, _i32, _i32, _i32, _f32, _vp]),
    "vd_attn_bwd": (C.c_int, [_vp, _vp, _vp, _i64, _vp, _i64, _vp, _i64, _vp, _vp, _vp, _vp, _vp, _i64, _i32, _i32, _i32, _i32, _f32, _vp]),
    "vd_attn_bwd_phase": (C.c_int, [_vp, _vp, _vp, _i64, _vp, _i64, _vp, _i64, _vp, _vp, _vp, _vp, _vp, _i64, _i32, _i32, _i32, _i32, _f32,
                                    _i32, _vp]),
    "vd_nchw_to_nhwc": (C.c_int, [_vp, _vp, _i32, _i32, _i32, _i32, _i64, _vp]),
    "vd_nhwc_to_nchw": (C.c_int, [_vp, _i64, _vp, _i32, _i32, _i32, _i32, _vp]),
    "vd_images_to_uint8_hwc": (C.c_int, [_vp, _vp, _i32, _i32, _i32, _vp]),
    "vd_images_from_uint8_hwc": (C.c_int, [_vp, _vp, _vp, _i32, _i32, _i32, _i32, _vp]),
    "vd_timestep_embedding": (C.c_int, [_vp, _vp, _i32, _i32, _f64, _vp]),
    "vd_class_embed": (C.c_int, [_vp, _vp, _vp, _vp, _i32, _i32, _i32, _vp]),
    "vd_class_embed_bwd": (C.c_int, [_vp, _vp, _vp, _vp, _i32, _i32, _i32, _i32, _vp]),
    "vd_multitag_norm": (C.c_int, [_vp, _vp, _i32, _i32, _vp]),
    "vd_im2col3x3": (C.c_int, [_vp, _i64, _vp, _i32, _i32, _i32, _i32, _vp]),
    "vd_tap_gather": (C.c_int, [_vp, _i64, _vp, _vp, _i64, _i32, _i32, _i32, _i32, _vp]),
    "vd_tap_spread": (C.c_int, [_vp, _i64, _vp, _i64, _i32, _i32, _i32, _i32, _vp]),
    "vd_thin_wgrad_finish": (C.c_int, [_vp, _i32, _i32, _i32, _vp, _i32, _vp, _i32, _i32, _vp, _vp]),
    "vd_q_sample": (C.c_int, [_vp, _vp, _vp, _vp, _i32, _i32, _i32, _vp]),
    "vd_loss_fwd": (C.c_int, [_vp, _vp, _vp, _vp, _vp, _i32, _i32, _vp, _vp, _i32, _i32, _i32, _vp]),
    "vd_loss_bwd": (C.c_int, [_vp, _vp, _vp, _vp, _vp, _vp, _vp, _i32, _i32, _vp, _i32, _i32, _i32, _vp]),
# ... 271 lines not shown
def wino43_pack(w, Cout, Cin, U43):
    _check(lib().vd_wino43_pack(ptr(w), Cout, Cin, ptr(U43), stream()), "vd_wino43_pack")


def wino43_pack_batched(table, n, total_blocks):
    assert table.is_cuda and table.dtype == torch.int64 and table.is_contiguous()
    _check(lib().vd_wino43_pack_batched(table.data_ptr(), n, total_blocks, stream()), "vd_wino43_pack_batched")


WINO43_FWD = os.environ.get("VD_WINO43_FWD", "1") != "0"


def wino43_fwd_supported(nimg, H, W, Cin, Cout, ldx, ldy, ldres=0):
    return (WINO and WINO43_FWD and bool(lib().vd_conv3x3_wino43_fwd_supported(nimg, H, W, Cin, Cout, ldx, ldy, ldres))
            and wino43_preferred(nimg, H, W, Cout))


def wino43_pack_fwd(w, Cout, Cin, U43f):
    _check(lib().vd_wino43_pack_fwd(ptr(w), Cout, Cin, ptr(U43f), stream()), "vd_wino43_pack_fwd")


def wino43_fwd_chunk_rows(H, W):
    return int(lib().vd_conv3x3_wino43_fwd_chunk_rows(H, W))


def conv3x3_wino43_fwd(x, ldx, U43f, bias, y, ldy, nimg, H, W, Cin, Cout, res=None, ldres=0, stats_part=None):
    name = f"wino43_conv_kernel<{W // 4}, true>"
    with _TimedName(name, 2.0 * nimg * H * W * Cout * 9 * Cin):
        _check(lib().vd_conv3x3_wino43_fwd(ptr(x), ldx, ptr(U43f), ptr(bias), ptr(res), ldres, ptr(y), ldy, nimg, H, W, Cin, Cout,
                                           ptr(stats_part), stream()), "vd_conv3x3_wino43_fwd")
    _note_bytes(name, 4.0 * (nimg * H * W * (Cin + Cout + (Cout if res is not None else 0)) + 36 * Cout * Cin))


def conv3x3_dgrad_wino43(dy, lddy, U43, dx, lddx, nimg, H, W, Cin, Cout):
    with _TimedName(f"wino43_conv_kernel<{W // 4}, false>", 2.0 * nimg * H * W * Cout * 9 * Cin):
        _check(lib().vd_conv3x3_dgrad_wino43(ptr(dy), lddy, ptr(U43), ptr(dx), lddx, nimg, H, W, Cin, Cout, stream()),
               "vd_conv3x3_dgrad_wino43")
    _note_bytes(f"wino43_conv_kernel<{W // 4}, false>", 4.0 * (nimg * H * W * (Cin + Cout) + 36 * Cout * Cin))


def conv3x3(x, ldx, wpack, bias, y, ldy, nimg, H, W, Cin, Cout, res=None, ldres=0, accumulate=False, stats_part=None):
    with _TimedTile("gemm_dma_kernel<{tile}, 2, 0, false, {kt}>", 2.0 * nimg * H * W * Cout * 9 * Cin):
        _check(lib().vd_conv3x3(ptr(x), ldx, ptr(wpack), ptr(bias), ptr(res), ldres, ptr(y), ldy, nimg, H, W, Cin, Cout,
                                int(accumulate), ptr(stats_part), stream()), "vd_conv3x3")


def conv3x3_wgrad_wino(x, ldx, dy, lddy, nimg, H, W, Cin, Cout, dw, Cin_w, Cout_w, accumulate=False, dbias=None):
    nb = lib().vd_conv3x3_wgrad_wino_ws_bytes(nimg, H, W, Cin, Cout)
    ws = workspace(nb, x.device, "wgrad")
    args = _wgrad_args(x, ldx, dy, lddy, nimg, H, W, Cin, Cout, dw, dbias, Cin_w, Cout_w, accumulate, ws)
    if PROFILE is None:
        _check(lib().vd_conv3x3_wgrad_wino(*args, stream()), "vd_conv3x3_wgrad_wino")
        return
    tws = min(W // 2, 16)
    with _TimedName(f"wino_wgrad_kernel<{tws}, {'true' if dbias is not None else 'false'}>", 2.0 * nimg * H * W * Cout * 9 * Cin):
        _check(lib().vd_conv3x3_wgrad_wino_phase(*args, 1, stream()), "vd_conv3x3_wgrad_wino_phase")
    with _TimedName("wino_wgrad_reduce_kernel", 0.0):
        _check(lib().vd_conv3x3_wgrad_wino_phase(*args, 2, stream()), "vd_conv3x3_wgrad_wino_phase")


WGRAD_STREAM = os.environ.get("VD_WGRAD_STREAM", "1") != "0"
GROUPED_AUTO_SPLIT = os.environ.get("VD_GROUPED_AUTO_SPLIT", "1") != "0"
GN_FOLD = os.environ.get("VD_GN_FOLD", "1") != "0"
GN_FOLD_MAX_CHUNKS = int(os.environ.get("VD_GN_FOLD_MAX_CHUNKS", "8"))
READY_PER_BLOCK = os.environ.get("VD_READY_PER_BLOCK", "0") != "0"
AUTOGRAD_CHAIN = os.environ.get("VD_AUTOGRAD_CHAIN", "1") != "0"
WINO43_WGRAD = os.environ.get("VD_WINO43_WGRAD", "1") != "0"
WINO43_WGRAD_MIN_TILES = int(os.environ.get("VD_WINO43_WGRAD_MIN_TILES", "512"))


W43_WGRAD_TAG = "[36 planes of the F(4x4,3x3) weight gradient]"


def wgrad43_supported(nimg, H, W, Cin, Cout, ldx, lddy):
    return (WINO and WINO43_WGRAD and nimg * (H // 4) * (W // 4) >= WINO43_WGRAD_MIN_TILES
            and bool(lib().vd_conv3x3_wgrad_wino43_supported(nimg, H, W, Cin, Cout, ldx, lddy)))


def conv3x3_wgrad_wino43(x, ldx, dy, lddy, nimg, H, W, Cin, Cout, dw, Cin_w, Cout_w, accumulate=False, dbias=None):
    nb = lib().vd_conv3x3_wgrad_wino43_ws_bytes(nimg, H, W, Cin, Cout)
    ws = workspace(nb, x.device, "wgrad43")
    args = _wgrad_args(x, ldx, dy, lddy, nimg, H, W, Cin, Cout, dw, dbias, Cin_w, Cout_w, accumulate, ws)
    if PROFILE is None:
        _check(lib().vd_conv3x3_wgrad_wino43(*args, stream()), "vd_conv3x3_wgrad_wino43")
        return
    with _TimedBytes("wino43_wgrad_transform_kernel", 4.0 * nimg * H * W * (Cin + Cout) * (1 + 2.25)):
        _check(lib().vd_conv3x3_wgrad_wino43_phase(*args, 1, stream()), "vd_conv3x3_wgrad_wino43_phase")
    with _TimedTile("gemm_dma_kernel<{tile}, 1, 1, true, {kt}, true> " + W43_WGRAD_TAG, 2.0 * nimg * H * W * Cout * 9 * Cin) as t:
        _check(lib().vd_conv3x3_wgrad_wino43_phase(*args, 2, stream()), "vd_conv3x3_wgrad_wino43_phase")
    _note_bytes(PROFILE[-1][0], 4.0 * (36.0 * nimg * (H // 4) * (W // 4) * (Cin + Cout) + 36.0 * Cout * Cin))
    with _TimedName("wino43_wgrad_finish_kernel", 0.0):
        _check(lib().vd_conv3x3_wgrad_wino43_phase(*args, 4, stream()), "vd_conv3x3_wgrad_wino43_phase")


def conv3x3_wgrad(x, ldx, dy, lddy, nimg, H, W, Cin, Cout, dw, Cin_w, Cout_w, accumulate=False, dbias=None, direct=False):
    if not direct and wgrad43_supported(nimg, H, W, Cin, Cout, ldx, lddy):
        return conv3x3_wgrad_wino43(x, ldx, dy, lddy, nimg, H, W, Cin, Cout, dw, Cin_w, Cout_w, accumulate, dbias)
    if WINO and not direct and lib().vd_conv3x3_wgrad_wino_supported(nimg, H, W, Cin, Cout, ldx, lddy):
        return conv3x3_wgrad_wino(x, ldx, dy, lddy, nimg, H, W, Cin, Cout, dw, Cin_w, Cout_w, accumulate, dbias)
    nb = lib().vd_conv3x3_wgrad_ws_bytes(nimg, H, W, Cin, Cout)
    ws = workspace(nb, x.device, "wgrad")
    args = _wgrad_args(x, ldx, dy, lddy, nimg, H, W, Cin, Cout, dw, dbias, Cin_w, Cout_w, accumulate, ws)
    flops = 2.0 * nimg * H * W * Cout * 9 * Cin
    if PROFILE is None:
        _check(lib().vd_conv3x3_wgrad(*args, stream()), "vd_conv3x3_wgrad")
        return
    with _TimedTile("gemm_dma_kernel<{tile}, 1, 2, true, {kt}>", flops):
        _check(lib().vd_conv3x3_wgrad_phase(*args, 1, stream()), "vd_conv3x3_wgrad_phase")
    with _TimedTile("reduce_slabs_oihw_kernel", 0.0):
        _check(lib().vd_conv3x3_wgrad_phase(*args, 2, stream()), "vd_conv3x3_wgrad_phase")


def im2col3x3(x, ldx, xc, nimg, H, W, Cc):
    _check(lib().vd_im2col3x3(ptr(x), ldx, ptr(xc), nimg, H, W, Cc, stream()), "vd_im2col3x3")


def tap_gather(z, ldz, bias, out, ldo, nimg, H, W, Cout):
    _check(lib().vd_tap_gather(ptr(z), ldz, ptr(bias), ptr(out), ldo, nimg, H, W, Cout, stream()), "vd_tap_gather")


def tap_spread(dy, lddy, dz, ldz, nimg, H, W, Cout):
    _check(lib().vd_tap_spread(ptr(dy), lddy, ptr(dz), ldz, nimg, H, W, Cout, stream()), "vd_tap_spread")


def thin_wgrad_finish(g, Cout_w, Cin, Cin_w, dw, accumulate=False, colsum=None, cs_stride=1, cs_off=0, dbias=None):
# ... 8 lines not shown
def pack_conv3x3_batched(table, n, total_blocks):
    assert table.is_cuda and table.dtype == torch.int64 and table.is_contiguous()
    _check(lib().vd_pack_conv3x3_batched(table.data_ptr(), n, total_blocks, stream()), "vd_pack_conv3x3_batched")


def gn_stats(x, ldx, nimg, HW, Cc, stats, G=32, eps=1e-6):
    nb = lib().vd_gn_ws_bytes(nimg, HW, Cc)
    ws = workspace(nb, x.device, "gn")
    _check(lib().vd_gn_stats(ptr(x), ldx, nimg, HW, Cc, G, eps, ptr(stats), ws.data_ptr(), ws.numel() * 4, stream()),
           "vd_gn_stats")


def _gn_bwd_name():
    k = lib().vd_gn_bwd_last_kernel()
    if k > 0:
        split, k = k // 100000000, k % 100000000
        nt, k = k >= 1000000, k % 1000000
        return f"gn_bwd_fused_kernel<{k // 10000}, {k % 10000}, {'true' if nt else 'false'}, {'true' if split else 'false'}>"
    return "gn_bwd_apply_kernel (two-pass form)" if k < 0 else "gn_bwd_apply_kernel (resample)"


def gn_apply(x, ldx, stats, gamma, beta, film, act, p_drop, seed, resample, y, ldy, nimg, H, W, Cc, coef, G=32):
    with _TimedBytes("gn_apply_kernel" if gamma is not None else "gn_apply_kernel (resample)", 4.0 * nimg * Cc * (H * W + _resampled_hw(H, W, resample))):
        _gn_apply(x, ldx, stats, gamma, beta, film, act, p_drop, seed, resample, y, ldy, nimg, H, W, Cc, coef, G)


def gn_apply_from_partials(x, ldx, parts, gamma, beta, film, act, p_drop, seed, resample, y, ldy, nimg, H, W, Cc, coef, G=32, eps=1e-6):
    with _TimedBytes("gn_apply_kernel", 4.0 * nimg * Cc * (H * W + _resampled_hw(H, W, resample))):
        _check(lib().vd_gn_apply_from_partials(ptr(x), ldx, *_two_parts(parts), ptr(gamma), ptr(beta), ptr(film), int(act),
                                               float(p_drop), int(seed), resample, ptr(y), ldy, nimg, H, W, Cc, G, eps, ptr(coef), stream()),
               "vd_gn_apply_from_partials")


def _gn_apply(x, ldx, stats, gamma, beta, film, act, p_drop, seed, resample, y, ldy, nimg, H, W, Cc, coef, G=32):
    _check(lib().vd_gn_apply(ptr(x), ldx, ptr(stats), ptr(gamma), ptr(beta), ptr(film), int(act), float(p_drop), int(seed),
                             resample, ptr(y), ldy, nimg, H, W, Cc, G, ptr(coef), stream()), "vd_gn_apply")


def gn_apply_bwd(dy, lddy, x, ldx, coef, gamma, beta, film, act, p_drop, seed, resample, add, ldadd, dx, lddx,
                 accumulate_dx, dfilm, dgamma, dbeta, accumulate_params, nimg, H, W, Cc, G=32, pgb_keep=None):
    nb = lib().vd_gn_ws_bytes(nimg, H * W, Cc)
    ws = workspace(nb, dy.device, "gn")
    nbytes = 4.0 * nimg * Cc * (_resampled_hw(H, W, resample) + H * W * (1 + (gamma is not None) + (add is not None) + bool(accumulate_dx)))
    with _TimedBytes("gn_apply_bwd", nbytes, rename=_gn_bwd_name):
        if pgb_keep is not None:
            _check(lib().vd_gn_apply_bwd_keep(ptr(dy), lddy, ptr(x), ldx, ptr(coef), ptr(gamma), ptr(beta), ptr(film), int(act),
                                              float(p_drop), int(seed), resample, ptr(add), ldadd, ptr(dx), lddx, int(accumulate_dx),
                                              ptr(dfilm), ptr(pgb_keep), nimg, H, W, Cc, G, ws.data_ptr(), ws.numel() * 4, stream()),
                   "vd_gn_apply_bwd_keep")
        else:
            _gn_apply_bwd_call(dy, lddy, x, ldx, coef, gamma, beta, film, act, p_drop, seed, resample, add, ldadd, dx, lddx,
                               accumulate_dx, dfilm, dgamma, dbeta, accumulate_params, nimg, H, W, Cc, G, ws)


def gn_param_sums_batched(table, n, total_blocks):
    assert table.is_cuda and table.dtype == torch.int64 and table.is_contiguous()
    _check(lib().vd_gn_param_sums_batched(table.data_ptr(), n, total_blocks, stream()), "vd_gn_param_sums_batched")


def _gn_apply_bwd_call(dy, lddy, x, ldx, coef, gamma, beta, film, act, p_drop, seed, resample, add, ldadd, dx, lddx,
                       accumulate_dx, dfilm, dgamma, dbeta, accumulate_params, nimg, H, W, Cc, G, ws):
    _check(lib().vd_gn_apply_bwd(ptr(dy), lddy, ptr(x), ldx, ptr(coef), ptr(gamma), ptr(beta), ptr(film), int(act),
                                 float(p_drop), int(seed), resample, ptr(add), ldadd, ptr(dx), lddx, int(accumulate_dx),
                                 ptr(dfilm), ptr(dgamma), ptr(dbeta), int(accumulate_params), nimg, H, W, Cc, G,
                                 ws.data_ptr(), ws.numel() * 4, stream()), "vd_gn_apply_bwd")

# ... 239 lines not shown
```

v-diffusion-torch_amd/v_diffusion/engine.py:

```python
import collections
import contextlib
import math

import torch

from . import _hip as H

GROUPS = 32
EPS = 1e-6
THIN = 8


def _ld(t):
    return t.stride(2)


def _chk(t):
    B, Hh, Ww, C = t.shape
    ld = t.stride(2)
    assert t.stride(3) == 1 and t.stride(1) == Ww * ld and t.stride(0) == Hh * Ww * ld, "not an NHWC view"
    return B, Hh, Ww, C, ld


def _splitk(M, N, K):
# ... 148 lines not shown
                pre = b.prefix + (".0" if b.att is not None else "")
                grp = self.film_groups.setdefault(2 * b.cout, [])
                self.film_slot[pre] = (2 * b.cout, len(grp))
                grp.append(b.res)
        self._pack_lru = {}
        self._packs = None
        self._fixed = None
        self._norm_channels = sum(p.numel() for k, p in model.named_parameters()
                                  if k.endswith(".weight") and p.ndim == 1)
        self._pgb_arena = self._pgb_table = None
        self._side = self._side_stream = None
        self._wq = None
        self._active_run = None
        self._segments = None

    @staticmethod
    def _new(ref, *shape):
        return torch.empty(shape, dtype=torch.float32, device=ref.device)

    def _res_of(self, level, H0, W0):
        return H0 >> level, W0 >> level

    def _part(self, ref, nimg, HW, C):
        if HW % 32:
            return None
        return torch.empty(H.stats_part_numel(nimg, HW, C), dtype=torch.float32, device=ref.device)

    @staticmethod
    def _parts(part, C, HW, rows=None):
        if part is None:
            return None
        return [(part, C, HW // (rows or (H.last_row_tile() // 2)))]

    def _norm(self, x, x_parts, gn, film, act, p_drop, seed, rs, y, B, Hh, Ww, C):
        coef = self._new(x, B, 4, C)
        stats = None
        if x_parts is not None and H.GN_FOLD and max(k for _, _, k in x_parts) <= H.GN_FOLD_MAX_CHUNKS:
            H.gn_apply_from_partials(x, _ld(x), x_parts, gn.weight, gn.bias, film, act, p_drop, seed, rs, y, _ld(y), B, Hh, Ww, C, coef,
                                     GROUPS, EPS)
            return coef
        if x_parts is not None:
            H.gn_coef_from_partials(x_parts, B, Hh * Ww, gn.weight, gn.bias, film, coef, GROUPS, EPS)
        else:
            stats = self._new(x, B, GROUPS, 2)
            H.gn_stats(x, _ld(x), B, Hh * Ww, C, stats, GROUPS, EPS)
        H.gn_apply(x, _ld(x), stats, gn.weight, gn.bias, film, act, p_drop, seed, rs, y, _ld(y), B, Hh, Ww, C, coef, GROUPS)
        return coef

    def _wgrad(self, dy, x, dw, db, M, N, K, lda, ldb, ldc):
        if self._wq is None or not H.GROUPED_WGRAD:
            H.gemm(dy, x, dw, M, N, K, a_kind=H.COL, b_kind=H.COL, lda=lda, ldb=ldb, ldc=ldc, splitk=_splitk(M, N, K), colsum=db)
            return
        key = (M, N, K, lda, ldb, ldc, db is not None)
        q = self._wq.setdefault(key, [])
        q.append((dy, x, dw, db))
        if len(q) == H.GROUP_MAX:
            self._wgrad_flush_key(key)

    def _cwgrad(self, x, ldx, dy, lddy, *args, **kw):
        side = self._side
        if side is None:
            return H.conv3x3_wgrad(x, ldx, dy, lddy, *args, **kw)
        side.wait_stream(torch.cuda.current_stream())
        x.record_stream(side)
        dy.record_stream(side)
        with torch.cuda.stream(side):
            H.conv3x3_wgrad(x, ldx, dy, lddy, *args, **kw)

    def _side_join(self):
        if self._side is not None:
            torch.cuda.current_stream().wait_stream(self._side)

    def _wgrad_flush_key(self, key):
        q = self._wq.pop(key, None)
        if not q:
            return
        M, N, K, lda, ldb, ldc, _ = key
        ok = M % 4 == 0 and N % 4 == 0 and lda % 4 == 0 and ldb % 4 == 0 and max(lda, ldb, ldc) * 128 + 128 < 0x70000000 // 4 and \
            all(dy.data_ptr() % 16 == 0 and x.data_ptr() % 16 == 0 for dy, x, _, _ in q)
        if len(q) == 1 or not ok:
            for dy, x, dw, db in q:
                H.gemm(dy, x, dw, M, N, K, a_kind=H.COL, b_kind=H.COL, lda=lda, ldb=ldb, ldc=ldc, splitk=_splitk(M, N, K), colsum=db)
            return
        if H.GROUPED_AUTO_SPLIT:
            S = H.lib().vd_gemm_grouped_wgrad_auto_split(len(q), M, N, K, 1, 64)
        else:
            tiles = ((M + 63) // 64) * ((N + 63) // 64) * len(q)
            S = max(1, min(64, 1024 // max(tiles, 1), K // 256))
        H.gemm_grouped_wgrad(q, M, N, K, lda, ldb, ldc, S)

    def _wgrad_flush(self):
        if not self._wq:
            return
        side = self._side
        if side is None:
            for key in list(self._wq):
                self._wgrad_flush_key(key)
            return
        side.wait_stream(torch.cuda.current_stream())
        for q in self._wq.values():
# ... 55 lines not shown
    @property
    def packs(self):
        return self._packs

    @contextlib.contextmanager
    def fixed_weights(self):
        self._fixed = {}
        try:
            yield
        finally:
            self._fixed = None

    def _layer(self, w):
        return self._packs.layers.get(id(w), _NO_PACK) if self._packs is not None else _NO_PACK

    def _conv(self, x, ldx, w, bias, y, ldy, B, Hh, Ww, Cin, Cout, dgrad=False, res=None, ldres=0, stats_part=None):
        pk, p = self._packs, self._layer(w)
        if not dgrad and p.u43f is not None and H.wino43_fwd_supported(B, Hh, Ww, Cin, Cout, ldx, ldy, ldres if res is not None else 0):
            H.conv3x3_wino43_fwd(x, ldx, p.u43f, bias, y, ldy, B, Hh, Ww, Cin, Cout, res=res, ldres=ldres, stats_part=stats_part)
            return H.wino43_fwd_chunk_rows(Hh, Ww)
        if dgrad and p.u43 is not None and H.wino43_supported(B, Hh, Ww, Cout, Cin, ldx, ldy):
            assert res is None and bias is None and stats_part is None
            H.conv3x3_dgrad_wino43(x, ldx, p.u43, y, ldy, B, Hh, Ww, Cout, Cin)
            return None
        if p is not _NO_PACK and pk.wino and H.wino_supported(B, Hh, Ww, Cin, Cout, ldx, ldy, ldres if res is not None else 0):
            U = p.ud if dgrad else p.uf
            if U is None:
                U = pk.image(w, dgrad)
            H.conv3x3_wino(x, ldx, U, bias, y, ldy, B, Hh, Ww, Cin, Cout, res=res, ldres=ldres, stats_part=stats_part)
            return H.last_row_tile() // 2
        H.conv3x3(x, ldx, self._pack_d(w) if dgrad else self._pack_f(w), bias, y, ldy, B, Hh, Ww, Cin, Cout, res=res, ldres=ldres,
                  stats_part=stats_part)
        return H.last_row_tile() // 2

    def _pack_f(self, w, cin_p=None):
        p = self._layer(w)
        if p.wf is not None:
            return p.wf
        cache = self._fixed
        if cache is not None and id(w) in cache:
            return cache[id(w)]
        co, ci = w.shape[0], w.shape[1]
        cin_p = cin_p or ci
        wf = self._new(w, co, 9, cin_p)
        H.pack_conv3x3(w, co, ci, wf=wf, Cin_p=cin_p)
        if cache is not None:
            cache[id(w)] = wf
        return wf

    def _pack_d(self, w, cout_p=None):
        p = self._layer(w)
        if p.wd is not None:
            return p.wd
        co, ci = w.shape[0], w.shape[1]
        cout_p = cout_p or co
        wd = self._new(w, ci, 9, cout_p)
        H.pack_conv3x3(w, co, ci, wd=wd, Cout_p=cout_p)
        return wd

    def _pack_thin(self, w, rows):
        cache = self._fixed
        key = ("thin", id(w))
        if cache is not None and key in cache:
            return cache[key]
        co, ci = w.shape[0], w.shape[1]
        wz = torch.zeros((rows, ci), dtype=torch.float32, device=w.device)
# ... 77 lines not shown
        films, stacks = {}, {}
        cache = self._fixed
        for c2, mods in self.film_groups.items():
            key = ("film", c2)
            if cache is not None and key in cache:
                W, bv = cache[key]
            else:
                W = torch.stack([mm.fc.weight.detach() for mm in mods])
                bv = torch.stack([mm.fc.bias.detach() for mm in mods])
                if cache is not None:
                    cache[key] = (W, bv)
            nb = len(mods)
            out = self._new(ta, nb, B, c2)
            H.gemm(ta, W, out, B, c2, E, a_kind=H.ROW, b_kind=H.ROW, lda=E, ldb=E, ldc=c2, bias=bv, sBias=c2, batch=nb,
                   sA=(0, 0), sB=(c2 * E, 0), sC=(B * c2, 0))
            films[c2], stacks[c2] = out, W
        if tape is not None:
            tape["film_w"] = stacks
        return films

    def _film_bwd(self, dfilms, stacks, dta):
        B, E = dta.shape
        for c2, df in dfilms.items():
            nb, W = df.shape[0], stacks[c2]
            P = self._new(dta, nb, B * E)
            H.gemm(df, W, P, B, E, c2, a_kind=H.ROW, b_kind=H.COL, lda=c2, ldb=E, ldc=E, batch=nb, sA=(B * c2, 0), sB=(c2 * E, 0),
                   sC=(B * E, 0))
            H.colsum(P, B * E, nb, B * E, dta.view(-1), accumulate=True)

    def _res_fwd(self, blk, mod, prefix, x, films, dest, p_drop, seed, tape, x_parts=None):
        B, Hh, Ww, Cin, ldx = _chk(x)
        Cout, rs = blk.cout, blk.rs
        Ho, Wo = (Hh // 2, Ww // 2) if rs == H.RS_DOWN else ((Hh * 2, Ww * 2) if rs == H.RS_UP else (Hh, Ww))
        a1 = self._new(x, B, Ho, Wo, Cin)
        coef1 = self._norm(x, x_parts, mod.norm1, None, 1, 0.0, 0, rs, a1, B, Hh, Ww, Cin)
        h1 = self._new(x, B, Ho, Wo, Cout)
        ph = self._part(x, B, Ho * Wo, Cout)
        rows = self._conv(a1, Cin, mod.conv1.weight, mod.conv1.bias, h1, Cout, B, Ho, Wo, Cin, Cout, stats_part=ph)
        h1_parts = self._parts(ph, Cout, Ho * Wo, rows)
        c2, fi = self.film_slot[prefix]
        film = films[c2][fi]
        a2 = self._new(x, B, Ho, Wo, Cout)
        coef2 = self._norm(h1, h1_parts, mod.norm2, film, 1, p_drop, seed, H.RS_NONE, a2, B, Ho, Wo, Cout)
        if rs != H.RS_NONE:
            xs = self._new(x, B, Ho, Wo, Cin)
            H.gn_apply(x, ldx, None, None, None, None, 0, 0.0, 0, rs, xs, Cin, B, Hh, Ww, Cin, None, GROUPS)
        else:
            xs = x
        has_skip = Cin != Cout
        if has_skip:
            sk = self._new(x, B, Ho, Wo, Cout)
            w = mod.skip.weight
            H.gemm(xs, w, sk, B * Ho * Wo, Cout, Cin, a_kind=H.ROW, b_kind=H.ROW, lda=_ld(xs), ldb=Cin, ldc=Cout, bias=mod.skip.bias)
        else:
            sk = xs
        pd = self._part(x, B, Ho * Wo, Cout)
        rows = self._conv(a2, Cout, mod.conv2.weight, mod.conv2.bias, dest, _ld(dest), B, Ho, Wo, Cout, Cout, res=sk,
                          ldres=_ld(sk), stats_part=pd)
        out_parts = self._parts(pd, Cout, Ho * Wo, rows)
        if tape is not None:
            tape[prefix] = dict(x=x, coef1=coef1, a1=a1, h1=h1, coef2=coef2, a2=a2, film=film, xs=xs if has_skip else None,
                                seed=seed, p=p_drop)
        return out_parts

    def _res_bwd(self, blk, mod, prefix, ctx, dy, dx, dx_accumulate, ta, dfilms, G):
        x, a1, h1, a2, film = ctx["x"], ctx["a1"], ctx["h1"], ctx["a2"], ctx["film"]
        B, Hh, Ww, Cin, ldx = _chk(x)
        _, Ho, Wo, Cout, lddy = _chk(dy)
        rs = blk.rs
        self._cwgrad(a2, Cout, dy, lddy, B, Ho, Wo, Cout, Cout, G[prefix + ".conv2.weight"], Cout, Cout,
                        dbias=G[prefix + ".conv2.bias"])
        da2 = self._new(x, B, Ho, Wo, Cout)
        self._conv(dy, lddy, mod.conv2.weight, None, da2, Cout, B, Ho, Wo, Cout, Cout, dgrad=True)
        dh1 = self._new(x, B, Ho, Wo, Cout)
        c2, fi = self.film_slot[prefix]
        dfilm = dfilms[c2][fi]
        H.gn_apply_bwd(da2, Cout, h1, Cout, ctx["coef2"], mod.norm2.weight, mod.norm2.bias, film, 1, ctx["p"], ctx["seed"],
                       H.RS_NONE, None, 0, dh1, Cout, False, dfilm, None, None, False, B, Ho, Wo, Cout, GROUPS,
                       pgb_keep=self._pgb(B, Cout, G[prefix + ".norm2.weight"], G[prefix + ".norm2.bias"]))
        del da2
        self._cwgrad(a1, Cin, dh1, Cout, B, Ho, Wo, Cin, Cout, G[prefix + ".conv1.weight"], Cin, Cout,
                        dbias=G[prefix + ".conv1.bias"])
        da1 = self._new(x, B, Ho, Wo, Cin)
        self._conv(dh1, Cout, mod.conv1.weight, None, da1, Cin, B, Ho, Wo, Cout, Cin, dgrad=True)
        del dh1
        if Cin != Cout:
            xs = ctx["xs"]
            P = B * Ho * Wo
            w = mod.skip.weight
            self._wgrad(dy, xs, G[prefix + ".skip.weight"], G[prefix + ".skip.bias"], Cout, Cin, P, lddy, _ld(xs), Cin)
            dsk = self._new(x, B, Ho, Wo, Cin)
            H.gemm(dy, w, dsk, P, Cin, Cout, a_kind=H.ROW, b_kind=H.COL, lda=lddy, ldb=Cin, ldc=Cin)
        else:
            dsk = dy
        if rs != H.RS_NONE:
            addt = self._new(x, B, Hh, Ww, Cin)
            H.gn_apply_bwd(dsk, _ld(dsk), None, 0, None, None, None, None, 0, 0.0, 0, rs, None, 0, addt, Cin, False, None, None,
                           None, False, B, Hh, Ww, Cin, GROUPS)
        else:
            addt = dsk
        H.gn_apply_bwd(da1, Cin, x, ldx, ctx["coef1"], mod.norm1.weight, mod.norm1.bias, None, 1, 0.0, 0, rs, addt, _ld(addt),
                       dx, _ld(dx), dx_accumulate, None, None, None, False, B, Hh, Ww, Cin, GROUPS,
                       pgb_keep=self._pgb(B, Cin, G[prefix + ".norm1.weight"], G[prefix + ".norm1.bias"]))
        self._linear_bwd(ta, mod.fc.weight, dfilm, G[prefix + ".fc.weight"], G[prefix + ".fc.bias"], None)

    def _attn_fwd(self, mod, prefix, x, dest, tape, x_parts=None):
        B, Hh, Ww, C, ldx = _chk(x)
        L, nh, hd = Hh * Ww, mod.num_heads, mod.head_dim
        hid = nh * hd
        xn = self._new(x, B, Hh, Ww, C)
        coef = self._norm(x, x_parts, mod.norm, None, 0, 0.0, 0, H.RS_NONE, xn, B, Hh, Ww, C)
        qkv = self._new(x, B, L, 3 * hid)
        H.gemm(xn, mod.proj_in.weight, qkv, B * L, 3 * hid, C, a_kind=H.ROW, b_kind=H.ROW, lda=C, ldb=C, ldc=3 * hid,
               bias=mod.proj_in.bias)
        ld = 3 * hid
# ... 351 lines not shown
```

Before: 2171.

## Emit Winograd-transformed activations directly from GroupNorm apply and reuse in wgrad

GroupNorm apply can now write the Winograd F(4,3) input transform V directly, in an octet-blocked layout, instead of the normalized NHWC activation. The forward conv then consumes V through a new fwd_v entry point, and the weight-gradient path reuses the same stored V through an octet-aware grouped wgrad GEMM. This removes the separate input transform in both the forward and wgrad convolutions and one NHWC activation round trip. In exchange the saved activation is 2.25x larger, which raises memory traffic and footprint for the backward pass.

```diff
diff --git a/include/vdiff_hip.h b/include/vdiff_hip.h
--- a/include/vdiff_hip.h
+++ b/include/vdiff_hip.h
@@ -90,6 +90,10 @@
 int vd_conv3x3_wino43_fwd_chunk_rows(int32_t H, int32_t W);
 int vd_conv3x3_wino43_fwd(const float* xin, int64_t ldx, const float* U43f, const float* bias, const float* res, int64_t ldres, float* y,
                           int64_t ldy, int32_t nimg, int32_t H, int32_t W, int32_t Cin, int32_t Cout, float* stats_part, void* stream);
+int vd_conv3x3_wino43_fwd_v_supported(int32_t nimg, int32_t H, int32_t W, int32_t Cin, int32_t Cout, int64_t ldy, int64_t ldres);
+size_t vd_wino43_v_floats(int32_t nimg, int32_t H, int32_t W, int32_t C);
+int vd_conv3x3_wino43_fwd_v(const float* V, const float* U43f, const float* bias, const float* res, int64_t ldres, float* y, int64_t ldy,
+                            int32_t nimg, int32_t H, int32_t W, int32_t Cin, int32_t Cout, float* stats_part, void* stream);
 int vd_conv3x3_wgrad_wino43_supported(int32_t nimg, int32_t H, int32_t W, int32_t Cin, int32_t Cout, int64_t ldx, int64_t lddy);
 size_t vd_conv3x3_wgrad_wino43_ws_bytes(int32_t nimg, int32_t H, int32_t W, int32_t Cin, int32_t Cout);
 int vd_conv3x3_wgrad_wino43(const float* xin, int64_t ldx, const float* dy, int64_t lddy, int32_t nimg, int32_t H, int32_t W,
@@ -98,6 +102,10 @@
 int vd_conv3x3_wgrad_wino43_phase(const float* xin, int64_t ldx, const float* dy, int64_t lddy, int32_t nimg, int32_t H, int32_t W,
                                   int32_t Cin, int32_t Cout, float* dw_oihw, float* dbias, int32_t Cin_w, int32_t Cout_w,
                                   int32_t accumulate, float* ws, size_t ws_bytes, int32_t phase, void* stream);
+size_t vd_conv3x3_wgrad_wino43_v_ws_bytes(int32_t nimg, int32_t H, int32_t W, int32_t Cin, int32_t Cout);
+int vd_conv3x3_wgrad_wino43_v(const float* V, const float* dy, int64_t lddy, int32_t nimg, int32_t H, int32_t W, int32_t Cin, int32_t Cout,
+                              float* dw_oihw, float* dbias, int32_t Cin_w, int32_t Cout_w, int32_t accumulate, float* ws, size_t ws_bytes,
+                              int32_t phases, void* stream);
 int vd_wino43_wgrad_last_kernel(void);
 
 int vd_wino_pack_batched(const int64_t* items_dev, int32_t n, int64_t total_blocks, void* stream);
@@ -145,6 +153,12 @@
                               uint64_t seed, int32_t resample, float* y, int64_t ldy, int32_t nimg, int32_t H, int32_t W, int32_t C,
                               int32_t G, float eps, float* coef, void* stream);
 
+int vd_gn_apply_v(const float* x, int64_t ldx, const float* stats, const float* gamma, const float* beta, const float* film, int32_t act,
+                  float p_drop, uint64_t seed, float* V, int32_t nimg, int32_t H, int32_t W, int32_t C, int32_t G, float* coef, void* stream);
+int vd_gn_apply_v_from_partials(const float* x, int64_t ldx, const float* part1, int32_t C1, int32_t chunks1, const float* part2, int32_t C2,
+                                int32_t chunks2, const float* gamma, const float* beta, const float* film, int32_t act, float p_drop,
+                                uint64_t seed, float* V, int32_t nimg, int32_t H, int32_t W, int32_t C, int32_t G, float eps, float* coef,
+                                void* stream);
 int vd_gn_apply_bwd(const float* dy, int64_t lddy, const float* x, int64_t ldx, const float* coef,
                     const float* gamma, const float* beta, const float* film, int32_t act, float p_drop, uint64_t seed,
                     int32_t resample, const float* add, int64_t ldadd, float* dx, int64_t lddx, int32_t accumulate_dx,
diff --git a/v-diffusion-torch_amd/csrc/common.h b/v-diffusion-torch_amd/csrc/common.h
--- a/v-diffusion-torch_amd/csrc/common.h
+++ b/v-diffusion-torch_amd/csrc/common.h
@@ -20,7 +20,7 @@
 int vd_persistent_cus(void);
 int vd_gemm_grouped_wgrad_kblk(const float* const* A, const float* const* B, float* const* C, float* const* colsum, int32_t count, int32_t M,
                                int32_t N, int32_t K, int64_t lda, int64_t ldb, int64_t ldc, int32_t splitk, float* ws, size_t ws_bytes,
-                               void* stream, int64_t a_kblk, int64_t b_kblk, int32_t slabs_only);
+                               void* stream, int64_t a_kblk, int64_t b_kblk, int32_t slabs_only, int64_t b_oct = 0);
 int vd_gemm_grouped_wgrad_used_slabs(int32_t count, int32_t M, int32_t N, int32_t K, int32_t splitk);
 extern thread_local int vd_g_last_tile;
 inline int vd_tile_code(bool tr, bool spl, int kt, int bm, int bn) {
@@ -59,3 +59,24 @@
     for (int j = 0; j < 4; ++j) m[j] = ((r[j] >> 8) * (1.0f / 16777216.0f) >= p) ? inv : 0.0f;
     return m;
 }
+
+__device__ __forceinline__ void bt6(const f32x4 (&d)[6], f32x4 (&o)[6]) {
+    const f32x4 e1 = d[4] - 2.25f * d[2], f1 = 0.75f * d[3] - 1.6875f * d[1];
+    const f32x4 e2 = d[4] - 0.5625f * d[2], f2 = 1.5f * d[3] - 0.84375f * d[1];
+    o[0] = 1.265625f * d[0] + (d[4] - 2.8125f * d[2]);
+    o[1] = e1 + f1;
+    o[2] = e1 - f1;
+    o[3] = e2 + f2;
+    o[4] = e2 - f2;
+    o[5] = 1.265625f * d[1] + (d[5] - 2.8125f * d[3]);
+}
+__device__ __forceinline__ void a6(const f32x4 (&y)[4], f32x4 (&o)[6]) {
+    const f32x4 e1 = y[0] + 0.5625f * y[2], f1 = 0.75f * y[1] + 0.421875f * y[3];
+    const f32x4 e2 = y[0] + 2.25f * y[2], f2 = 1.5f * y[1] + 3.375f * y[3];
+    o[0] = y[0];
+    o[1] = e1 + f1;
+    o[2] = e1 - f1;
+    o[3] = e2 + f2;
+    o[4] = e2 - f2;
+    o[5] = y[3];
+}
diff --git a/v-diffusion-torch_amd/csrc/gemm.hip b/v-diffusion-torch_amd/csrc/gemm.hip
--- a/v-diffusion-torch_amd/csrc/gemm.hip
+++ b/v-diffusion-torch_amd/csrc/gemm.hip
@@ -27,6 +27,7 @@
     int group_S;
     int lgW, lgHW;
     long long a_kblk, b_kblk;
+    long long b_oct;
 };
 
 __device__ __forceinline__ int PB(const GemmArgs& p) { return VD_PROBE_BUILD ? p.probe : 0; }
@@ -471,13 +472,14 @@
             kcB[j] = kk;
             const bool ok = (BK == VD_IM2COL) ? (ci0 + cn < p.Cin) : (n0 + cn < p.N);
             const int rowoff = (GROUPED && BK == VD_COL && p.b_kblk) ? (kk >> 4) * (int)p.b_kblk + (kk & 15) * (int)p.ldb : kk * (int)p.ldb;
-            voB[j] = ok ? (unsigned)(rowoff + cn) * 4u : OOB;
+            const int coloff = (GROUPED && BK == VD_COL && p.b_oct) ? (cn >> 3) * (int)p.b_oct + (cn & 7) : cn;
+            voB[j] = ok ? (unsigned)(rowoff + coloff) * 4u : OOB;
             if (BK == VD_IM2COL) pix_yx(p, kt_begin * KT + kk, by[j], bx[j]);
             else by[j] = bx[j] = 0;
         }
     }
     const float* Ablk = (AK == VD_COL) ? A + m0 : A + (long long)m0 * p.lda;
-    const float* Bblk = (BK == VD_ROW) ? B + (long long)n0 * p.ldb : ((BK == VD_COL) ? B + n0 : B + ci0);
+    const float* Bblk = (BK == VD_ROW) ? B + (long long)n0 * p.ldb : ((BK == VD_COL) ? ((GROUPED && p.b_oct) ? B + (n0 >> 3) * p.b_oct : B + n0) : B + ci0);
     const long long tapoffB = (BK == VD_IM2COL) ? (long long)((tapN / 3 - 1) * p.W + (tapN % 3 - 1)) * p.ldb : 0;
 
 #ifndef VD_ISSUE_IN
@@ -943,7 +945,8 @@
     const int m0 = tby * BM, n0 = tbx * BN;
     const int e = tbz / p.group_S, slab = tbz - e * p.group_S;
     const float* A = gp.A[e] + m0;
-    const float* B = gp.B[e] + n0;
+    const float* B = gp.B[e] + (p.b_oct ? (n0 >> 3) * p.b_oct : (long long)n0);
+    const int boffB = p.b_oct ? ((lane >> 1) * (int)p.b_oct + (lane & 1) * 4) * 4 : lane * 16;
     const int kt_begin = slab * p.kt_per_split, kt_end = min(kt_begin + p.kt_per_split, p.kt_total);
     float* C = p.C + (long long)tbz * p.slab_stride;
 
@@ -957,7 +960,7 @@
         for (int h = 0; h < 2; ++h) {
             const int kk = wave + 8 * h;
             __builtin_amdgcn_raw_ptr_buffer_load_lds(rsA, (lds_ptr_t)(as + kk * BM), 16, lane * 16, kk * (int)p.lda * 4, 0, 0);
-            __builtin_amdgcn_raw_ptr_buffer_load_lds(rsB, (lds_ptr_t)(bs + kk * BN), 16, lane * 16, kk * (int)p.ldb * 4, 0, 0);
+            __builtin_amdgcn_raw_ptr_buffer_load_lds(rsB, (lds_ptr_t)(bs + kk * BN), 16, boffB, kk * (int)p.ldb * 4, 0, 0);
         }
     };
 
@@ -1424,7 +1427,7 @@
 extern "C" int vd_gemm_grouped_wgrad(const float* const* A, const float* const* B, float* const* C, float* const* colsum, int32_t count,
                                      int32_t M, int32_t N, int32_t K, int64_t lda, int64_t ldb, int64_t ldc, int32_t splitk, float* ws,
                                      size_t ws_bytes, void* stream) {
-    return vd_gemm_grouped_wgrad_kblk(A, B, C, colsum, count, M, N, K, lda, ldb, ldc, splitk, ws, ws_bytes, stream, 0, 0, 0);
+    return vd_gemm_grouped_wgrad_kblk(A, B, C, colsum, count, M, N, K, lda, ldb, ldc, splitk, ws, ws_bytes, stream, 0, 0, 0, 0);
 }
 
 int vd_gemm_grouped_wgrad_used_slabs(int32_t count, int32_t M, int32_t N, int32_t K, int32_t splitk) {
@@ -1433,7 +1436,7 @@
 
 int vd_gemm_grouped_wgrad_kblk(const float* const* A, const float* const* B, float* const* C, float* const* colsum, int32_t count,
                                int32_t M, int32_t N, int32_t K, int64_t lda, int64_t ldb, int64_t ldc, int32_t splitk, float* ws,
-                               size_t ws_bytes, void* stream, int64_t a_kblk, int64_t b_kblk, int32_t slabs_only) {
+                               size_t ws_bytes, void* stream, int64_t a_kblk, int64_t b_kblk, int32_t slabs_only, int64_t b_oct) {
     VD_REQUIRE(A && B && C && count > 0 && count <= VD_GROUP_MAX, "vd_gemm_grouped_wgrad: 1..%d entries (got %d)", VD_GROUP_MAX, count);
     VD_REQUIRE(M > 0 && N > 0 && K > 0 && M % 4 == 0 && N % 4 == 0 && lda % 4 == 0 && ldb % 4 == 0 && ldc >= N,
                "vd_gemm_grouped_wgrad: M, N, lda, ldb must be multiples of 4 (M=%d N=%d)", M, N);
@@ -1449,7 +1452,9 @@
     a.A = A[0]; a.B = B[0];
     a.M = M; a.N = N; a.K = K; a.lda = lda; a.ldb = ldb; a.ldc = N; a.ldr = 0; a.nh = 1;
     a.alpha = 1.f; a.lgW = a.lgHW = -1; a.probe = 0;
-    a.a_kblk = a_kblk; a.b_kblk = b_kblk;
+    a.a_kblk = a_kblk; a.b_kblk = b_kblk; a.b_oct = b_oct;
+    VD_REQUIRE(b_oct == 0 || (ldb == 8 && b_kblk > 0 && N % 8 == 0 && b_oct % 4 == 0 && (long long)(N / 8) * b_oct + 2 * b_kblk + 128 < 0x70000000LL / 4),
+               "vd_gemm_grouped_wgrad: octet-blocked B needs ldb = 8, K blocks and N %% 8 == 0");
     VD_REQUIRE(a_kblk >= 0 && b_kblk >= 0 && a_kblk % 4 == 0 && b_kblk % 4 == 0 && 2 * a_kblk + 16 * lda + 128 < 0x70000000LL / 4 &&
                2 * b_kblk + 16 * ldb + 128 < 0x70000000LL / 4, "vd_gemm_grouped_wgrad: K-block strides outside the LDS-DMA kernel's range");
     VD_REQUIRE(dma_in_range(a), "vd_gemm_grouped_wgrad: operands outside the LDS-DMA kernel's range (alignment / row pitch)");
diff --git a/v-diffusion-torch_amd/csrc/norm.hip b/v-diffusion-torch_amd/csrc/norm.hip
--- a/v-diffusion-torch_amd/csrc/norm.hip
+++ b/v-diffusion-torch_amd/csrc/norm.hip
@@ -335,6 +335,96 @@
     }
 }
 
+constexpr int VOCT = 36 * 16 * 8;
+template <bool FROM_PARTS>
+__global__ __launch_bounds__(256) void gn_apply_v_kernel(const ApplyArgs p, const PartArgs q, float* V, int TW, int TPI) {
+    __shared__ double ps[FROM_PARTS ? 2 : 1][FROM_PARTS ? 256 : 1];
+    __shared__ float gst[FROM_PARTS ? 2 : 1][FROM_PARTS ? 68 : 1];
+    const int tid = threadIdx.x, lane = tid & 63, wave = tid >> 6;
+    const int c0 = blockIdx.y * 64;
+    const int oct = (c0 >> 3) + 2 * wave + (lane >> 5), c4 = oct * 8 + (lane & 1) * 4;
+    const int tile = blockIdx.x * 16 + ((lane >> 1) & 15);
+    const int b = (blockIdx.x * 16) / TPI;
+    const bool active = c4 < p.C;
+    f32x4 sc = {1.f, 1.f, 1.f, 1.f}, of = {0.f, 0.f, 0.f, 0.f};
+    if (FROM_PARTS) {
+        const int C = p.C, cg = C / q.G;
+        const int g0 = c0 / cg, g1 = (min(c0 + 64, C) - 1) / cg, cb0 = g0 * cg, nc = (g1 + 1) * cg - cb0;
+        for (int cl = tid; cl < nc; cl += 256) {
+            const int c = cb0 + cl;
+            const bool first = c < q.C1;
+            const int Cs = first ? q.C1 : q.C2, cs = first ? c : c - q.C1, chunks = first ? q.ch1 : q.ch2;
+            const float* src = (first ? q.p1 : q.p2) + (long long)b * chunks * 2 * Cs + cs;
+            double s1 = 0.0, s2 = 0.0;
+            for (int ch = 0; ch < chunks; ++ch) { s1 += (double)src[(long long)ch * 2 * Cs]; s2 += (double)src[(long long)ch * 2 * Cs + Cs]; }
+            ps[0][cl] = s1; ps[1][cl] = s2;
+        }
+        __syncthreads();
+        for (int g = tid; g <= g1 - g0; g += 256) {
+            double s1 = 0.0, s2 = 0.0;
+            for (int c = g * cg; c < (g + 1) * cg; ++c) { s1 += ps[0][c]; s2 += ps[1][c]; }
+            const double n = (double)cg * (double)p.H * (double)p.W;
+            const double mean = s1 / n;
+            double var = s2 / n - mean * mean;
+            if (var < 0.0) var = 0.0;
+            gst[0][g] = (float)mean; gst[1][g] = (float)(1.0 / sqrt(var + (double)q.eps));
+        }
+        __syncthreads();
+        if (!active) return;
+        f32x4 nr, nm;
+#pragma unroll
+        for (int j = 0; j < 4; ++j) {
+            const int c = c4 + j, g = c / cg - g0;
+            const float mean = gst[0][g], rstd = gst[1][g];
+            float s_ = rstd * q.gamma[c];
+            float o_ = q.beta[c] - mean * s_;
+            if (q.film) {
+                const float shift = q.film[(long long)b * 2 * C + c], scale = q.film[(long long)b * 2 * C + C + c];
+                s_ *= (1.f + scale);
+                o_ = o_ * (1.f + scale) + shift;
+            }
+            sc[j] = s_; of[j] = o_; nr[j] = rstd; nm[j] = -mean * rstd;
+        }
+        if (tile == b * TPI && q.coef_out) {
+            float* o = q.coef_out + (long long)b * 4 * C + c4;
+            *reinterpret_cast<f32x4*>(o) = sc; *reinterpret_cast<f32x4*>(o + C) = of;
+            *reinterpret_cast<f32x4*>(o + 2 * C) = nr; *reinterpret_cast<f32x4*>(o + 3 * C) = nm;
+        }
+    } else {
+        if (!active) return;
+        if (p.has_norm) {
+            const float* cf = p.coef + (long long)b * 4 * p.C;
+            sc = *reinterpret_cast<const f32x4*>(cf + c4);
+            of = *reinterpret_cast<const f32x4*>(cf + p.C + c4);
+        }
+    }
+    const int tin = tile - b * TPI, ty = tin / TW, tx = tin - ty * TW;
+    const float* ximg = p.x + (long long)b * p.H * p.W * p.ldx;
+    f32x4 R[6][6];
+#pragma unroll
+    for (int pr = 0; pr < 6; ++pr) {
+        const int yy = 4 * ty - 1 + pr;
+        f32x4 d[6];
+#pragma unroll
+        for (int qx = 0; qx < 6; ++qx) {
+            const int xx = 4 * tx - 1 + qx;
+            d[qx] = f32x4{0.f, 0.f, 0.f, 0.f};
+            if ((unsigned)yy < (unsigned)p.H && (unsigned)xx < (unsigned)p.W) d[qx] = fwd_one(p, ximg, yy * p.W + xx, c4, sc, of, b);
+        }
+        bt6(d, R[pr]);
+    }
+    float* vb = V + ((long long)blockIdx.x * (p.C >> 3) + oct) * VOCT + ((lane >> 1) & 15) * 8 + (lane & 1) * 4;
+#pragma unroll
+    for (int bb = 0; bb < 6; ++bb) {
+        f32x4 col[6], o[6];
+#pragma unroll
+        for (int pr = 0; pr < 6; ++pr) col[pr] = R[pr][bb];
+        bt6(col, o);
+#pragma unroll
+        for (int a = 0; a < 6; ++a) *reinterpret_cast<f32x4*>(vb + (6 * a + bb) * 128) = o[a];
+    }
+}
+
 __global__ __launch_bounds__(256) void gn_bwd_finalize_kernel(const float* part, int chunks, const float* coef,
                                                               const float* gamma, const float* beta, const float* film,
                                                               int C, int G, long long HW, float* q, float* dfilm,
@@ -843,6 +933,55 @@
                "vd_gn_apply_from_partials: cannot split C=%d into whole-group channel ranges", C);
     hipLaunchKernelGGL(gn_apply_kernel<true>, dim3((unsigned)((Ho * Wo + APIX - 1) / APIX), nimg, C / Cba), dim3(256), 0, st, p, Cba, q);
     VD_LAUNCH_CHECK("gn_apply_kernel<from partials>");
+    return 0;
+}
+
+static int gn_apply_v_check(const char* who, const float* x, int64_t ldx, float* V, int32_t nimg, int32_t H, int32_t W, int32_t C) {
+    VD_REQUIRE(x && V && vd_aligned16(x) && vd_aligned16(V), "%s: null / unaligned operand", who);
+    VD_REQUIRE(nimg > 0 && H > 0 && W > 0 && H % 4 == 0 && W % 4 == 0 && ((H / 4) * (W / 4)) % 16 == 0 && C % 8 == 0 && ldx % 4 == 0 && ldx >= C,
+               "%s: needs whole blocks of 16 tiles per image and C %% 8 == 0 (H=%d W=%d C=%d)", who, H, W, C);
+    VD_REQUIRE((long long)nimg * H * W < (1LL << 31) / 2 && (long long)H * W * ldx < (1LL << 31), "%s: tensor too large", who);
+    return 0;
+}
+
+extern "C" int vd_gn_apply_v(const float* x, int64_t ldx, const float* stats, const float* gamma, const float* beta, const float* film,
+                             int32_t act, float p_drop, uint64_t seed, float* V, int32_t nimg, int32_t H, int32_t W, int32_t C, int32_t G,
+                             float* coef, void* stream) {
+    hipStream_t st = (hipStream_t)stream;
+    if (gn_apply_v_check("vd_gn_apply_v", x, ldx, V, nimg, H, W, C)) return 1;
+    const int has_norm = gamma != nullptr;
+    if (has_norm && !stats) {
+        VD_REQUIRE(coef != nullptr, "vd_gn_apply_v: neither statistics nor a coefficient table given");
+    } else if (has_norm) {
+        VD_REQUIRE(stats && beta && coef && C % G == 0, "vd_gn_apply_v: missing norm operands");
+        hipLaunchKernelGGL(gn_coef_kernel, dim3((nimg * C + 255) / 256), dim3(256), 0, st, stats, gamma, beta, film, nimg, C, G, coef);
+        VD_LAUNCH_CHECK("gn_coef_kernel");
+    }
+    VD_REQUIRE(!has_norm || vd_aligned16(coef), "vd_gn_apply_v: coefficient table must be 16-byte aligned");
+    ApplyArgs p = {x, ldx, coef, has_norm, act, p_drop, seed, VD_RS_NONE, nullptr, 0, nimg, H, W, C};
+    const int TPI = (H / 4) * (W / 4);
+    hipLaunchKernelGGL(gn_apply_v_kernel<false>, dim3((unsigned)(nimg * (TPI / 16)), (unsigned)((C + 63) / 64)), dim3(256), 0, st, p, PartArgs{}, V,
+                       W / 4, TPI);
+    VD_LAUNCH_CHECK("gn_apply_v_kernel");
+    return 0;
+}
+
+extern "C" int vd_gn_apply_v_from_partials(const float* x, int64_t ldx, const float* part1, int32_t C1, int32_t chunks1, const float* part2,
+                                           int32_t C2, int32_t chunks2, const float* gamma, const float* beta, const float* film, int32_t act,
+                                           float p_drop, uint64_t seed, float* V, int32_t nimg, int32_t H, int32_t W, int32_t C, int32_t G,
+                                           float eps, float* coef, void* stream) {
+    hipStream_t st = (hipStream_t)stream;
+    if (gn_apply_v_check("vd_gn_apply_v_from_partials", x, ldx, V, nimg, H, W, C)) return 1;
+    VD_REQUIRE(part1 && gamma && beta, "vd_gn_apply_v_from_partials: null operand");
+    VD_REQUIRE(G > 0 && C % G == 0 && C1 + C2 == C && C1 > 0 && chunks1 > 0, "vd_gn_apply_v_from_partials: bad channel split C=%d C1=%d C2=%d G=%d", C, C1, C2, G);
+    VD_REQUIRE(C2 == 0 || (part2 && chunks2 > 0), "vd_gn_apply_v_from_partials: second source incomplete");
+    VD_REQUIRE(!coef || vd_aligned16(coef), "vd_gn_apply_v_from_partials: coefficient table must be 16-byte aligned");
+    VD_REQUIRE(64 + 2 * (C / G) <= 256, "vd_gn_apply_v_from_partials: groups of %d channels are too wide", C / G);
+    ApplyArgs p = {x, ldx, coef, 1, act, p_drop, seed, VD_RS_NONE, nullptr, 0, nimg, H, W, C};
+    PartArgs q = {part1, C1, chunks1, part2, C2, chunks2, G, eps, gamma, beta, film, coef};
+    const int TPI = (H / 4) * (W / 4);
+    hipLaunchKernelGGL(gn_apply_v_kernel<true>, dim3((unsigned)(nimg * (TPI / 16)), (unsigned)((C + 63) / 64)), dim3(256), 0, st, p, q, V, W / 4, TPI);
+    VD_LAUNCH_CHECK("gn_apply_v_kernel<from partials>");
     return 0;
 }
 
diff --git a/v-diffusion-torch_amd/csrc/wino43.hip b/v-diffusion-torch_amd/csrc/wino43.hip
--- a/v-diffusion-torch_amd/csrc/wino43.hip
+++ b/v-diffusion-torch_amd/csrc/wino43.hip
@@ -85,8 +85,9 @@
 template <bool DY>
 __device__ __forceinline__ void bt_full2(const f32x2 (&r)[6], f32x2 (&v)[6]) { bt_full<DY, f32x2>(r, v); }
 
-template <int TWT, bool FWD>
+template <int TWT, bool FWD, bool VIN = false>
 __global__ __launch_bounds__(THREADS) void wino43_conv_kernel(const Args43 p) {
+    static_assert(!VIN || (FWD && TWT <= 8 && 3 * (18 - SB_STEP) == 18), "the V-input form exists for the forward pass on 32x32 and 16x16 images");
     constexpr bool QUAD = TWT == 4;
     constexpr int RUN = TWT + 1;
     constexpr int RUNS = QUAD ? 4 * RUN - 2 : 4 * RUN;
@@ -162,14 +163,14 @@
         } else {
             const int j = i - 5;
             const int s = (wave >> 1) + 4 * j, g = wave & 1;
-            if (s < NPG) {
+            if (!VIN && s < NPG) {
                 const __amdgpu_buffer_rsrc_t rs = make_rsrc(xitem + kt * KT);
                 __builtin_amdgcn_raw_ptr_buffer_load_lds(rs, (lds_ptr_t)(sb + (g * NPG + s) * 256), 16, (int)pxo[j], g * 16, 0, 0);
             }
         }
     };
-    constexpr int NPIECE = 5 + APL;
-    constexpr int SB = SB_STEP, NAFTER = 18 - SB, PAFTER = NAFTER;
+    constexpr int NPIECE = VIN ? 5 : 5 + APL;
+    constexpr int SB = SB_STEP, NAFTER = 18 - SB, PAFTER = VIN ? 5 : NAFTER;
     constexpr int UPF = U_AHEAD;
     static_assert(PAFTER <= NPIECE && NPIECE - PAFTER <= SB, "DMA schedule does not fit the tile");
 
@@ -210,13 +211,14 @@
             }
         };
         auto first_stage = [&](int cbx, int grpx) {
-            if (QUAD) xitem = p.x + (long long)grpx * (4 * 16 * 16) * p.ldx;
+            if constexpr (VIN) {}
+            else if (QUAD) xitem = p.x + (long long)grpx * (4 * 16 * 16) * p.ldx;
             else { offsets(grpx); xitem = p.x + (long long)(grpx / p.items_per_img) * p.H * p.W * p.ldx; }
 #pragma unroll
             for (int i = 0; i < NPIECE; ++i) issue_piece(i, 0, 0, cbx);
         };
         int cb = 0, grp = 0, cb_next = 0, grp_next = 0;
-        if (QUAD) offsets(0);
+        if (QUAD && !VIN) offsets(0);
         bool have = item_of(0, cb, grp);
         if (have) first_stage(cb, grp);
         for (int n = 0; have; ++n) {
@@ -226,65 +228,117 @@
             f32x4 acc[18][2];
 #pragma unroll
             for (int x = 0; x < 18; ++x) { acc[x][0] = f32x4{0.f, 0.f, 0.f, 0.f}; acc[x][1] = f32x4{0.f, 0.f, 0.f, 0.f}; }
-            if (n == 0) asm volatile("s_waitcnt vmcnt(0)" ::: "memory");
-            else asm volatile("s_waitcnt vmcnt(16)" ::: "memory");
-            lds_barrier();
-            stamp(1);
-            if (nkt > 1) {
-#pragma unroll
-                for (int i = 0; i < PAFTER; ++i) issue_piece(i, 1, 1, cb);
-            }
-            f32x2 R[3][6];
-            rowpass(smem + pbase, R, 0, 6);
-            stamp(2);
-            for (int kt = 0; kt < nkt; ++kt) {
-                const int st = kt & 1;
-                const float* su = smem + st * STAGE + uoff;
-                const float* san = smem + (st ^ 1) * STAGE + pbase;
-                const bool n1 = kt + 1 < nkt, n2 = kt + 2 < nkt;
-                f32x2 Rn[3][6];
-                f32x4 uf[UPF + 1], ufl[NAFTER];
-#pragma unroll
-                for (int e = 0; e < UPF; ++e) uf[e] = *reinterpret_cast<const f32x4*>(su + (18 * HALF + e) * 256);
-#pragma unroll
-                for (int a = 0; a < 3; ++a) {
-                    f32x2 V[6];
-                    bt_full2<FWD>(R[a], V);
-#pragma unroll
-                    for (int b = 0; b < 6; ++b) {
-                        const int xl = 6 * a + b;
+            if constexpr (VIN) {
+                const float* vitem = p.x + (long long)(4 * grp + tg) * nkt * (36 * 16 * KT);
+                const int voff = (li * KT + 2 * lq) * 4;
+                f32x2 Vc[18];
+                {
+                    const __amdgpu_buffer_rsrc_t rv = make_rsrc(vitem);
+#pragma unroll
+                    for (int x = 0; x < 18; ++x)
+                        Vc[x] = __builtin_bit_cast(f32x2, __builtin_amdgcn_raw_buffer_load_b64(rv, voff, (18 * HALF + x) * 16 * KT * 4, 0));
+                }
+                asm volatile("s_waitcnt vmcnt(0)" ::: "memory");
+                lds_barrier();
+                stamp(1);
+                if (nkt > 1) {
+#pragma unroll
+                    for (int i = 0; i < PAFTER; ++i) issue_piece(i, 1, 1, cb);
+                }
+                stamp(2);
+                for (int kt = 0; kt < nkt; ++kt) {
+                    const int st = kt & 1;
+                    const float* su = smem + st * STAGE + uoff;
+                    const bool n1 = kt + 1 < nkt, n2 = kt + 2 < nkt;
+                    const __amdgpu_buffer_rsrc_t rv = make_rsrc(vitem + (long long)(n1 ? kt + 1 : kt) * (36 * 16 * KT), n1 ? (int)OOB : 0);
+                    f32x4 uf[UPF + 1], ufl[NAFTER];
+#pragma unroll
+                    for (int e = 0; e < UPF; ++e) uf[e] = *reinterpret_cast<const f32x4*>(su + (18 * HALF + e) * 256);
+#pragma unroll
+                    for (int xl = 0; xl < 18; ++xl) {
                         if (xl == SB) {
 #pragma unroll
                             for (int e = 0; e < NAFTER; ++e) ufl[e] = *reinterpret_cast<const f32x4*>(su + (18 * HALF + SB + e) * 256);
-                            if (VD_PROBE_BUILD && p.probe) {
-                                const unsigned long long ta = __builtin_amdgcn_s_memtime();
-                                asm volatile("s_waitcnt vmcnt(0)" ::: "memory");
-                                const unsigned long long tb = __builtin_amdgcn_s_memtime();
-                                __syncthreads();
-                                const unsigned long long tc = __builtin_amdgcn_s_memtime();
-                                t_vm += tb - ta; t_bar += tc - tb;
-                            } else {
-                                asm volatile("s_waitcnt vmcnt(0)" ::: "memory");
-                                __syncthreads();
+                            asm volatile("s_waitcnt vmcnt(0)" ::: "memory");
+                            lds_barrier();
+                        }
+                        if (xl + UPF < SB) uf[(xl + UPF) % (UPF + 1)] = *reinterpret_cast<const f32x4*>(su + (18 * HALF + xl + UPF) * 256);
+                        if (xl >= SB && xl - SB < PAFTER) { if (n2) issue_piece(xl - SB, kt + 2, st, cb); }
+                        const f32x4 u = xl < SB ? uf[xl % (UPF + 1)] : ufl[xl < SB ? 0 : xl - SB];
+                        acc[xl][0] = __builtin_amdgcn_mfma_f32_16x16x4f32(u[0], Vc[xl][0], acc[xl][0], 0, 0, 0);
+                        acc[xl][1] = __builtin_amdgcn_mfma_f32_16x16x4f32(u[2], Vc[xl][0], acc[xl][1], 0, 0, 0);
+                        acc[xl][0] = __builtin_amdgcn_mfma_f32_16x16x4f32(u[1], Vc[xl][1], acc[xl][0], 0, 0, 0);
+                        acc[xl][1] = __builtin_amdgcn_mfma_f32_16x16x4f32(u[3], Vc[xl][1], acc[xl][1], 0, 0, 0);
+                        if (xl >= SB) {
+#pragma unroll
+                            for (int j = 0; j < 3; ++j) {
+                                const int x = j < 2 ? 2 * (xl - SB) + j : xl;
+                                Vc[x] = __builtin_bit_cast(f32x2, __builtin_amdgcn_raw_buffer_load_b64(rv, voff, (18 * HALF + x) * 16 * KT * 4, 0));
                             }
                         }
-                        if (xl + UPF < SB) uf[(xl + UPF) % (UPF + 1)] = *reinterpret_cast<const f32x4*>(su + (18 * HALF + xl + UPF) * 256);
-                        if (xl + PAFTER < NPIECE) { if (n1) issue_piece(xl + PAFTER, kt + 1, st ^ 1, cb); }
-                        if (xl >= SB) {
-                            if (n2) issue_piece(xl - SB, kt + 2, st, cb);
-                            rowpass(san, Rn, (6 * (xl - SB)) / NAFTER, (6 * (xl - SB + 1)) / NAFTER);
+                    }
+                }
+            } else {
+                if (n == 0) asm volatile("s_waitcnt vmcnt(0)" ::: "memory");
+                else asm volatile("s_waitcnt vmcnt(16)" ::: "memory");
+                lds_barrier();
+                stamp(1);
+                if (nkt > 1) {
+    #pragma unroll
+                    for (int i = 0; i < PAFTER; ++i) issue_piece(i, 1, 1, cb);
+                }
+                f32x2 R[3][6];
+                rowpass(smem + pbase, R, 0, 6);
+                stamp(2);
+                for (int kt = 0; kt < nkt; ++kt) {
+                    const int st = kt & 1;
+                    const float* su = smem + st * STAGE + uoff;
+                    const float* san = smem + (st ^ 1) * STAGE + pbase;
+                    const bool n1 = kt + 1 < nkt, n2 = kt + 2 < nkt;
+                    f32x2 Rn[3][6];
+                    f32x4 uf[UPF + 1], ufl[NAFTER];
+    #pragma unroll
+                    for (int e = 0; e < UPF; ++e) uf[e] = *reinterpret_cast<const f32x4*>(su + (18 * HALF + e) * 256);
+    #pragma unroll
+                    for (int a = 0; a < 3; ++a) {
+                        f32x2 V[6];
+                        bt_full2<FWD>(R[a], V);
+    #pragma unroll
+                        for (int b = 0; b < 6; ++b) {
+                            const int xl = 6 * a + b;
+                            if (xl == SB) {
+    #pragma unroll
+                                for (int e = 0; e < NAFTER; ++e) ufl[e] = *reinterpret_cast<const f32x4*>(su + (18 * HALF + SB + e) * 256);
+                                if (VD_PROBE_BUILD && p.probe) {
+                                    const unsigned long long ta = __builtin_amdgcn_s_memtime();
+                                    asm volatile("s_waitcnt vmcnt(0)" ::: "memory");
+                                    const unsigned long long tb = __builtin_amdgcn_s_memtime();
+                                    __syncthreads();
+                                    const unsigned long long tc = __builtin_amdgcn_s_memtime();
+                                    t_vm += tb - ta; t_bar += tc - tb;
+                                } else {
+                                    asm volatile("s_waitcnt vmcnt(0)" ::: "memory");
+                                    __syncthreads();
+                                }
+                            }
+                            if (xl + UPF < SB) uf[(xl + UPF) % (UPF + 1)] = *reinterpret_cast<const f32x4*>(su + (18 * HALF + xl + UPF) * 256);
+                            if (xl + PAFTER < NPIECE) { if (n1) issue_piece(xl + PAFTER, kt + 1, st ^ 1, cb); }
+                            if (xl >= SB) {
+                                if (n2) issue_piece(xl - SB, kt + 2, st, cb);
+                                rowpass(san, Rn, (6 * (xl - SB)) / NAFTER, (6 * (xl - SB + 1)) / NAFTER);
+                            }
+                            const f32x4 u = xl < SB ? uf[xl % (UPF + 1)] : ufl[xl < SB ? 0 : xl - SB];
+                            acc[xl][0] = __builtin_amdgcn_mfma_f32_16x16x4f32(u[0], V[b][0], acc[xl][0], 0, 0, 0);
+                            acc[xl][1] = __builtin_amdgcn_mfma_f32_16x16x4f32(u[2], V[b][0], acc[xl][1], 0, 0, 0);
+                            acc[xl][0] = __builtin_amdgcn_mfma_f32_16x16x4f32(u[1], V[b][1], acc[xl][0], 0, 0, 0);
+                            acc[xl][1] = __builtin_amdgcn_mfma_f32_16x16x4f32(u[3], V[b][1], acc[xl][1], 0, 0, 0);
                         }
-                        const f32x4 u = xl < SB ? uf[xl % (UPF + 1)] : ufl[xl < SB ? 0 : xl - SB];
-                        acc[xl][0] = __builtin_amdgcn_mfma_f32_16x16x4f32(u[0], V[b][0], acc[xl][0], 0, 0, 0);
-                        acc[xl][1] = __builtin_amdgcn_mfma_f32_16x16x4f32(u[2], V[b][0], acc[xl][1], 0, 0, 0);
-                        acc[xl][0] = __builtin_amdgcn_mfma_f32_16x16x4f32(u[1], V[b][1], acc[xl][0], 0, 0, 0);
-                        acc[xl][1] = __builtin_amdgcn_mfma_f32_16x16x4f32(u[3], V[b][1], acc[xl][1], 0, 0, 0);
                     }
-                }
-#pragma unroll
-                for (int a = 0; a < 3; ++a)
-#pragma unroll
-                    for (int q = 0; q < 6; ++q) R[a][q] = Rn[a][q];
+    #pragma unroll
+                    for (int a = 0; a < 3; ++a)
+    #pragma unroll
+                        for (int q = 0; q < 6; ++q) R[a][q] = Rn[a][q];
+                }
             }
             stamp(3);
             __syncthreads();
@@ -488,32 +542,12 @@
                 (int)((long long)blockIdx.x - it[7]), (int)it[2]);
 }
 
-__device__ __forceinline__ void bt6(const f32x4 (&d)[6], f32x4 (&o)[6]) {
-    const f32x4 e1 = d[4] - 2.25f * d[2], f1 = 0.75f * d[3] - 1.6875f * d[1];
-    const f32x4 e2 = d[4] - 0.5625f * d[2], f2 = 1.5f * d[3] - 0.84375f * d[1];
-    o[0] = 1.265625f * d[0] + (d[4] - 2.8125f * d[2]);
-    o[1] = e1 + f1;
-    o[2] = e1 - f1;
-    o[3] = e2 + f2;
-    o[4] = e2 - f2;
-    o[5] = 1.265625f * d[1] + (d[5] - 2.8125f * d[3]);
-}
-__device__ __forceinline__ void a6(const f32x4 (&y)[4], f32x4 (&o)[6]) {
-    const f32x4 e1 = y[0] + 0.5625f * y[2], f1 = 0.75f * y[1] + 0.421875f * y[3];
-    const f32x4 e2 = y[0] + 2.25f * y[2], f2 = 1.5f * y[1] + 3.375f * y[3];
-    o[0] = y[0];
-    o[1] = e1 + f1;
-    o[2] = e1 - f1;
-    o[3] = e2 + f2;
-    o[4] = e2 - f2;
-    o[5] = y[3];
-}
-
 __device__ __forceinline__ void st_once(float* p, f32x4 v) { *reinterpret_cast<f32x4*>(p) = v; }
 struct WgT43 {
     const float* x; long long ldx; const float* dy; long long lddy;
     float* V; float* dM;
     int nimg, H, W, Cin, Cout, TW, TPI, T;
+    int z0;
 };
 
 __global__ __launch_bounds__(256) void wino43_wgrad_transform_kernel(const WgT43 p) {
@@ -522,7 +556,7 @@
     const int img = tile / p.TPI, tin = tile - img * p.TPI;
     const int ty = tin / p.TW, tx = tin - ty * p.TW;
     const int c4 = 4 * quad;
-    if (blockIdx.z == 0) {
+    if (blockIdx.z + p.z0 == 0) {
         if (c4 >= p.Cin) return;
         f32x4 R[6][6];
 #pragma unroll
@@ -671,13 +705,13 @@
 }
 
 struct Wg43Plan { bool ok; int T, S; size_t v_f, m_f, u_f, cs_f, gemm_bytes; };
-Wg43Plan wg43_plan(int nimg, int H, int W, int Cin, int Cout) {
+Wg43Plan wg43_plan(int nimg, int H, int W, int Cin, int Cout, bool v_given = false) {
     Wg43Plan g = {};
     if (nimg <= 0 || H % 4 || W % 4 || H < 4 || W < 4 || Cin % 4 || Cout % 4) return g;
     g.T = nimg * (H / 4) * (W / 4);
     g.S = vd_gemm_grouped_wgrad_auto_split(36, Cout, Cin, g.T, (g.T + 1535) / 1536, 24);
     const size_t T16 = ((size_t)g.T + 15) / 16 * 16;
-    g.v_f = (size_t)36 * T16 * Cin; g.m_f = (size_t)36 * T16 * Cout; g.u_f = (size_t)36 * Cout * Cin; g.cs_f = (size_t)36 * Cout;
+    g.v_f = v_given ? 0 : (size_t)36 * T16 * Cin; g.m_f = (size_t)36 * T16 * Cout; g.u_f = (size_t)36 * Cout * Cin; g.cs_f = (size_t)36 * Cout;
     g.gemm_bytes = vd_gemm_grouped_wgrad_ws_bytes(36, Cout, Cin, g.S);
     g.ok = true;
     return g;
@@ -800,6 +834,45 @@
     return 0;
 }
 
+extern "C" int vd_conv3x3_wino43_fwd_v_supported(int32_t nimg, int32_t H, int32_t W, int32_t Cin, int32_t Cout, int64_t ldy, int64_t ldres) {
+    if (!((W == 32 && H == 32) || (W == 16 && H == 16))) return 0;
+    return vd_conv3x3_wino43_fwd_supported(nimg, H, W, Cin, Cout, Cin, ldy, ldres);
+}
+
+extern "C" size_t vd_wino43_v_floats(int32_t nimg, int32_t H, int32_t W, int32_t C) {
+    return (size_t)36 * nimg * (H / 4) * (W / 4) * C;
+}
+
+extern "C" int vd_conv3x3_wino43_fwd_v(const float* V, const float* U43f, const float* bias, const float* res, int64_t ldres, float* y,
+                                       int64_t ldy, int32_t nimg, int32_t H, int32_t W, int32_t Cin, int32_t Cout, float* stats_part,
+                                       void* stream) {
+    VD_REQUIRE(V && U43f && y, "vd_conv3x3_wino43_fwd_v: null operand");
+    VD_REQUIRE(vd_conv3x3_wino43_fwd_v_supported(nimg, H, W, Cin, Cout, ldy, res ? ldres : 0),
+               "vd_conv3x3_wino43_fwd_v: unsupported geometry nimg=%d H=%d W=%d Cin=%d Cout=%d", nimg, H, W, Cin, Cout);
+    VD_REQUIRE(vd_aligned16(V) && vd_aligned16(U43f) && vd_aligned16(y) && (!res || vd_aligned16(res)) && (!bias || vd_aligned16(bias)),
+               "vd_conv3x3_wino43_fwd_v: operands must be 16-byte aligned");
+    Args43 a = {};
+    a.x = V; a.ldx = Cin; a.U = U43f; a.y = y; a.ldy = ldy;
+    a.nimg = nimg; a.H = H; a.W = W; a.K = Cin; a.N = Cout;
+    a.items_per_img = 1;
+    a.ngrp = W == 16 ? nimg / 4 : nimg;
+    a.ncb = Cout / TN;
+    a.bias = bias; a.res = res; a.ldr = ldres; a.stats = stats_part;
+    a.chunks_per_img = 1;
+    const long long items = (long long)a.ngrp * a.ncb;
+    VD_REQUIRE(items < (1LL << 30), "vd_conv3x3_wino43_fwd_v: too many work items");
+    a.nitems = (int)items;
+    a.probe = g_probe43;
+    const int ncu = vd_persistent_cus();
+    const dim3 grid((unsigned)(items < ncu ? items : ncu)), blk(THREADS);
+    hipStream_t st = (hipStream_t)stream;
+    if (W == 16) hipLaunchKernelGGL((wino43_conv_kernel<4, true, true>), grid, blk, 0, st, a);
+    else hipLaunchKernelGGL((wino43_conv_kernel<8, true, true>), grid, blk, 0, st, a);
+    VD_LAUNCH_CHECK("wino43_conv_kernel<., true, true>");
+    g_last43 = -(100 + W / 4);
+    return 0;
+}
+
 extern "C" int vd_wino43_pack_batched(const int64_t* items_dev, int32_t n, int64_t total_blocks, void* stream) {
     VD_REQUIRE(items_dev && n > 0 && total_blocks > 0 && total_blocks < (1LL << 31), "vd_wino43_pack_batched: bad table");
     hipLaunchKernelGGL(wino43_pack_batched_kernel, dim3((unsigned)total_blocks), dim3(256), 0, (hipStream_t)stream,
@@ -825,14 +898,18 @@
 
 static int wgrad43_impl(const float* xin, int64_t ldx, const float* dy, int64_t lddy, int32_t nimg, int32_t H, int32_t W, int32_t Cin,
                         int32_t Cout, float* dw_oihw, float* dbias, int32_t Cin_w, int32_t Cout_w, int32_t accumulate, float* ws,
-                        size_t ws_bytes, void* stream, int phases) {
+                        size_t ws_bytes, void* stream, int phases, const float* vin = nullptr) {
+    if (vin) {
+        VD_REQUIRE(Cin % 8 == 0 && (nimg * (H / 4) * (W / 4)) % 16 == 0 && vd_aligned16(vin), "vd_conv3x3_wgrad_wino43_v: V needs Cin %% 8 == 0 and whole blocks of 16 tiles");
+        xin = vin; ldx = Cin;
+    }
     VD_REQUIRE(xin && dy && dw_oihw && ws, "vd_conv3x3_wgrad_wino43: null operand");
     VD_REQUIRE(vd_conv3x3_wgrad_wino43_supported(nimg, H, W, Cin, Cout, ldx, lddy),
                "vd_conv3x3_wgrad_wino43: unsupported geometry nimg=%d H=%d W=%d Cin=%d Cout=%d", nimg, H, W, Cin, Cout);
     VD_REQUIRE(Cin_w <= Cin && Cout_w <= Cout, "vd_conv3x3_wgrad_wino43: real dims exceed padded dims");
     VD_REQUIRE(vd_aligned16(xin) && vd_aligned16(dy) && vd_aligned16(ws), "vd_conv3x3_wgrad_wino43: operands must be 16-byte aligned");
-    VD_REQUIRE(ws_bytes >= vd_conv3x3_wgrad_wino43_ws_bytes(nimg, H, W, Cin, Cout), "vd_conv3x3_wgrad_wino43: workspace too small");
-    const Wg43Plan g = wg43_plan(nimg, H, W, Cin, Cout);
+    const Wg43Plan g = wg43_plan(nimg, H, W, Cin, Cout, vin != nullptr);
+    VD_REQUIRE(ws_bytes >= (g.v_f + g.m_f + g.u_f + g.cs_f) * sizeof(float) + g.gemm_bytes, "vd_conv3x3_wgrad_wino43: workspace too small");
     float* V = ws;
     float* dM = V + g.v_f;
     float* dU = dM + g.m_f;
@@ -843,19 +920,20 @@
         WgT43 t = {};
         t.x = xin; t.ldx = ldx; t.dy = dy; t.lddy = lddy; t.V = V; t.dM = dM;
         t.nimg = nimg; t.H = H; t.W = W; t.Cin = Cin; t.Cout = Cout; t.TW = W / 4; t.TPI = (H / 4) * (W / 4); t.T = g.T;
-        const int cmax = Cin > Cout ? Cin : Cout;
-        hipLaunchKernelGGL(wino43_wgrad_transform_kernel, dim3((unsigned)(g.T / 4), (unsigned)((cmax + 255) / 256), 2), dim3(64, 4), 0, st, t);
+        t.z0 = vin ? 1 : 0;
+        const int cmax = vin ? Cout : (Cin > Cout ? Cin : Cout);
+        hipLaunchKernelGGL(wino43_wgrad_transform_kernel, dim3((unsigned)(g.T / 4), (unsigned)((cmax + 255) / 256), vin ? 1 : 2), dim3(64, 4), 0, st, t);
         VD_LAUNCH_CHECK("wino43_wgrad_transform_kernel");
     }
     if (phases & 2) {
         const float* A[36]; const float* B[36]; float* C[36]; float* colsum[36];
         for (int e = 0; e < 36; ++e) {
-            A[e] = dM + (size_t)e * 16 * Cout; B[e] = V + (size_t)e * 16 * Cin;
+            A[e] = dM + (size_t)e * 16 * Cout; B[e] = vin ? vin + (size_t)e * 16 * 8 : V + (size_t)e * 16 * Cin;
             C[e] = dU + (size_t)e * Cout * Cin; colsum[e] = cs + (size_t)e * Cout;
         }
-        const int rc = vd_gemm_grouped_wgrad_kblk(A, B, C, colsum, 36, Cout, Cin, g.T, Cout, Cin, Cin, g.S, gws, g.gemm_bytes, stream,
+        const int rc = vd_gemm_grouped_wgrad_kblk(A, B, C, colsum, 36, Cout, Cin, g.T, Cout, vin ? 8 : Cin, Cin, g.S, gws, g.gemm_bytes, stream,
                                                   36LL * 16 * Cout, 36LL * 16 * Cin,
-                                                  (long long)Cout * Cin >= FUSED_FINISH_MIN ? 1 : 0);
+                                                  (long long)Cout * Cin >= FUSED_FINISH_MIN ? 1 : 0, vin ? 36LL * 16 * 8 : 0);
         if (rc) return rc;
         g_last43w = g.S;
     }
@@ -887,4 +965,18 @@
     return wgrad43_impl(xin, ldx, dy, lddy, nimg, H, W, Cin, Cout, dw_oihw, dbias, Cin_w, Cout_w, accumulate, ws, ws_bytes, stream, phase);
 }
 
+extern "C" size_t vd_conv3x3_wgrad_wino43_v_ws_bytes(int32_t nimg, int32_t H, int32_t W, int32_t Cin, int32_t Cout) {
+    const Wg43Plan g = wg43_plan(nimg, H, W, Cin, Cout, true);
+    if (!g.ok) return 0;
+    return (g.m_f + g.u_f + g.cs_f) * sizeof(float) + g.gemm_bytes;
+}
+
+extern "C" int vd_conv3x3_wgrad_wino43_v(const float* V, const float* dy, int64_t lddy, int32_t nimg, int32_t H, int32_t W, int32_t Cin,
+                                         int32_t Cout, float* dw_oihw, float* dbias, int32_t Cin_w, int32_t Cout_w, int32_t accumulate,
+                                         float* ws, size_t ws_bytes, int32_t phases, void* stream) {
+    VD_REQUIRE(V != nullptr, "vd_conv3x3_wgrad_wino43_v: null V");
+    VD_REQUIRE(phases == 7 || phases == 1 || phases == 2 || phases == 4, "vd_conv3x3_wgrad_wino43_v: phases must be 7 (all), 1, 2 or 4");
+    return wgrad43_impl(nullptr, 0, dy, lddy, nimg, H, W, Cin, Cout, dw_oihw, dbias, Cin_w, Cout_w, accumulate, ws, ws_bytes, stream, phases, V);
+}
+
 extern "C" int vd_wino43_wgrad_last_kernel(void) { return g_last43w; }
diff --git a/v-diffusion-torch_amd/v_diffusion/_hip.py b/v-diffusion-torch_amd/v_diffusion/_hip.py
--- a/v-diffusion-torch_amd/v_diffusion/_hip.py
+++ b/v-diffusion-torch_amd/v_diffusion/_hip.py
@@ -58,11 +58,16 @@
     "vd_wino43_pack_fwd": (C.c_int, [_vp, _i32, _i32, _vp, _vp]),
     "vd_conv3x3_wino43_fwd_chunk_rows": (C.c_int, [_i32, _i32]),
     "vd_conv3x3_wino43_fwd": (C.c_int, [_vp, _i64, _vp, _vp, _vp, _i64, _vp, _i64, _i32, _i32, _i32, _i32, _i32, _vp, _vp]),
+    "vd_conv3x3_wino43_fwd_v_supported": (C.c_int, [_i32, _i32, _i32, _i32, _i32, _i64, _i64]),
+    "vd_wino43_v_floats": (_sz, [_i32, _i32, _i32, _i32]),
+    "vd_conv3x3_wino43_fwd_v": (C.c_int, [_vp, _vp, _vp, _vp, _i64, _vp, _i64, _i32, _i32, _i32, _i32, _i32, _vp, _vp]),
     "vd_wino43_pack": (C.c_int, [_vp, _i32, _i32, _vp, _vp]),
     "vd_wino43_pack_batched": (C.c_int, [_vp, _i32, _i64, _vp]),
     "vd_conv3x3_wgrad_wino43_supported": (C.c_int, [_i32, _i32, _i32, _i32, _i32, _i64, _i64]),
     "vd_conv3x3_wgrad_wino43_ws_bytes": (_sz, [_i32, _i32, _i32, _i32, _i32]),
     "vd_conv3x3_wgrad_wino43": (C.c_int, [_vp, _i64, _vp, _i64, _i32, _i32, _i32, _i32, _i32, _vp, _vp, _i32, _i32, _i32, _vp, _sz, _vp]),
+    "vd_conv3x3_wgrad_wino43_v_ws_bytes": (_sz, [_i32, _i32, _i32, _i32, _i32]),
+    "vd_conv3x3_wgrad_wino43_v": (C.c_int, [_vp, _vp, _i64, _i32, _i32, _i32, _i32, _i32, _vp, _vp, _i32, _i32, _i32, _vp, _sz, _i32, _vp]),
     "vd_wino43_wgrad_last_kernel": (C.c_int, []),
     "vd_conv3x3_wgrad_wino43_phase": (C.c_int, [_vp, _i64, _vp, _i64, _i32, _i32, _i32, _i32, _i32, _vp, _vp, _i32, _i32, _i32, _vp, _sz, _i32, _vp]),
     "vd_gn_stats_from_partials": (C.c_int, [_vp, _i32, _i32, _vp, _i32, _i32, _i32, _i32, _i32, _f32, _vp, _vp]),
@@ -77,6 +82,9 @@
     "vd_gn_apply": (C.c_int, [_vp, _i64, _vp, _vp, _vp, _vp, _i32, _f32, _u64, _i32, _vp, _i64, _i32, _i32, _i32, _i32, _i32, _vp, _vp]),
     "vd_gn_apply_from_partials": (C.c_int, [_vp, _i64, _vp, _i32, _i32, _vp, _i32, _i32, _vp, _vp, _vp, _i32, _f32, _u64, _i32, _vp, _i64, _i32,
                                             _i32, _i32, _i32, _i32, _f32, _vp, _vp]),
+    "vd_gn_apply_v": (C.c_int, [_vp, _i64, _vp, _vp, _vp, _vp, _i32, _f32, _u64, _vp, _i32, _i32, _i32, _i32, _i32, _vp, _vp]),
+    "vd_gn_apply_v_from_partials": (C.c_int, [_vp, _i64, _vp, _i32, _i32, _vp, _i32, _i32, _vp, _vp, _vp, _i32, _f32, _u64, _vp, _i32, _i32, _i32,
+                                              _i32, _i32, _f32, _vp, _vp]),
     "vd_gn_apply_bwd": (C.c_int, [_vp, _i64, _vp, _i64, _vp, _vp, _vp, _vp, _i32, _f32, _u64, _i32, _vp, _i64, _vp, _i64, _i32,
                                   _vp, _vp, _vp, _i32, _i32, _i32, _i32, _i32, _i32, _vp, _sz, _vp]),
     "vd_gn_bwd_last_kernel": (C.c_int, []),
@@ -414,6 +422,26 @@
     _note_bytes(name, 4.0 * (nimg * H * W * (Cin + Cout + (Cout if res is not None else 0)) + 36 * Cout * Cin))
 
 
+V_HANDOVER = os.environ.get("VD_V_HANDOVER", "0") != "0"
+
+
+def v_handover_supported(nimg, H, W, Cin, Cout, ldy, ldres=0):
+    return (V_HANDOVER and WINO and WINO43_FWD and bool(lib().vd_conv3x3_wino43_fwd_v_supported(nimg, H, W, Cin, Cout, ldy, ldres))
+            and wino43_preferred(nimg, H, W, Cout))
+
+
+def wino43_v_numel(nimg, H, W, Cc):
+    return 36 * nimg * (H // 4) * (W // 4) * Cc
+
+
+def conv3x3_wino43_fwd_v(V, U43f, bias, y, ldy, nimg, H, W, Cin, Cout, res=None, ldres=0, stats_part=None):
+    name = f"wino43_conv_kernel<{W // 4}, true, true>"
+    with _TimedName(name, 2.0 * nimg * H * W * Cout * 9 * Cin):
+        _check(lib().vd_conv3x3_wino43_fwd_v(ptr(V), ptr(U43f), ptr(bias), ptr(res), ldres, ptr(y), ldy, nimg, H, W, Cin, Cout,
+                                             ptr(stats_part), stream()), "vd_conv3x3_wino43_fwd_v")
+    _note_bytes(name, 4.0 * (nimg * H * W * (2.25 * Cin + Cout + (Cout if res is not None else 0)) + 36 * Cout * Cin))
+
+
 def conv3x3_dgrad_wino43(dy, lddy, U43, dx, lddx, nimg, H, W, Cin, Cout):
     with _TimedName(f"wino43_conv_kernel<{W // 4}, false>", 2.0 * nimg * H * W * Cout * 9 * Cin):
         _check(lib().vd_conv3x3_dgrad_wino43(ptr(dy), lddy, ptr(U43), ptr(dx), lddx, nimg, H, W, Cin, Cout, stream()),
@@ -473,6 +501,22 @@
     _note_bytes(PROFILE[-1][0], 4.0 * (36.0 * nimg * (H // 4) * (W // 4) * (Cin + Cout) + 36.0 * Cout * Cin))
     with _TimedName("wino43_wgrad_finish_kernel", 0.0):
         _check(lib().vd_conv3x3_wgrad_wino43_phase(*args, 4, stream()), "vd_conv3x3_wgrad_wino43_phase")
+
+
+def conv3x3_wgrad_wino43_v(V, dy, lddy, nimg, H, W, Cin, Cout, dw, Cin_w, Cout_w, accumulate=False, dbias=None):
+    nb = lib().vd_conv3x3_wgrad_wino43_v_ws_bytes(nimg, H, W, Cin, Cout)
+    ws = workspace(nb, V.device, "wgrad43")
+    args = (ptr(V), ptr(dy), lddy, nimg, H, W, Cin, Cout, ptr(dw), ptr(dbias), Cin_w, Cout_w, int(accumulate), ws.data_ptr(), ws.numel() * 4)
+    if PROFILE is None:
+        _check(lib().vd_conv3x3_wgrad_wino43_v(*args, 7, stream()), "vd_conv3x3_wgrad_wino43_v")
+        return
+    with _TimedBytes("wino43_wgrad_transform_kernel", 4.0 * nimg * H * W * Cout * (1 + 2.25)):
+        _check(lib().vd_conv3x3_wgrad_wino43_v(*args, 1, stream()), "vd_conv3x3_wgrad_wino43_v")
+    with _TimedTile("gemm_dma_kernel<{tile}, 1, 1, true, {kt}, true> " + W43_WGRAD_TAG, 2.0 * nimg * H * W * Cout * 9 * Cin):
+        _check(lib().vd_conv3x3_wgrad_wino43_v(*args, 2, stream()), "vd_conv3x3_wgrad_wino43_v")
+    _note_bytes(PROFILE[-1][0], 4.0 * (36.0 * nimg * (H // 4) * (W // 4) * (Cin + Cout) + 36.0 * Cout * Cin))
+    with _TimedName("wino43_wgrad_finish_kernel", 0.0):
+        _check(lib().vd_conv3x3_wgrad_wino43_v(*args, 4, stream()), "vd_conv3x3_wgrad_wino43_v")
 
 
 def conv3x3_wgrad(x, ldx, dy, lddy, nimg, H, W, Cin, Cout, dw, Cin_w, Cout_w, accumulate=False, dbias=None, direct=False):
@@ -547,6 +591,18 @@
                "vd_gn_apply_from_partials")
 
 
+def gn_apply_v(x, ldx, stats, gamma, beta, film, act, p_drop, seed, V, nimg, H, W, Cc, coef, G=32):
+    with _TimedBytes("gn_apply_v_kernel", 4.0 * nimg * Cc * H * W * (1 + 2.25)):
+        _check(lib().vd_gn_apply_v(ptr(x), ldx, ptr(stats), ptr(gamma), ptr(beta), ptr(film), int(act), float(p_drop), int(seed), ptr(V),
+                                   nimg, H, W, Cc, G, ptr(coef), stream()), "vd_gn_apply_v")
+
+
+def gn_apply_v_from_partials(x, ldx, parts, gamma, beta, film, act, p_drop, seed, V, nimg, H, W, Cc, coef, G=32, eps=1e-6):
+    with _TimedBytes("gn_apply_v_kernel", 4.0 * nimg * Cc * H * W * (1 + 2.25)):
+        _check(lib().vd_gn_apply_v_from_partials(ptr(x), ldx, *_two_parts(parts), ptr(gamma), ptr(beta), ptr(film), int(act), float(p_drop),
+                                                 int(seed), ptr(V), nimg, H, W, Cc, G, eps, ptr(coef), stream()), "vd_gn_apply_v_from_partials")
+
+
 def _gn_apply(x, ldx, stats, gamma, beta, film, act, p_drop, seed, resample, y, ldy, nimg, H, W, Cc, coef, G=32):
     _check(lib().vd_gn_apply(ptr(x), ldx, ptr(stats), ptr(gamma), ptr(beta), ptr(film), int(act), float(p_drop), int(seed),
                              resample, ptr(y), ldy, nimg, H, W, Cc, G, ptr(coef), stream()), "vd_gn_apply")
diff --git a/v-diffusion-torch_amd/v_diffusion/engine.py b/v-diffusion-torch_amd/v_diffusion/engine.py
--- a/v-diffusion-torch_amd/v_diffusion/engine.py
+++ b/v-diffusion-torch_amd/v_diffusion/engine.py
@@ -204,9 +204,21 @@
             return None
         return [(part, C, HW // (rows or (H.last_row_tile() // 2)))]
 
-    def _norm(self, x, x_parts, gn, film, act, p_drop, seed, rs, y, B, Hh, Ww, C):
+    def _norm(self, x, x_parts, gn, film, act, p_drop, seed, rs, y, B, Hh, Ww, C, v_out=False):
         coef = self._new(x, B, 4, C)
         stats = None
+        if v_out:
+            assert rs == H.RS_NONE
+            if x_parts is not None and H.GN_FOLD and max(k for _, _, k in x_parts) <= H.GN_FOLD_MAX_CHUNKS:
+                H.gn_apply_v_from_partials(x, _ld(x), x_parts, gn.weight, gn.bias, film, act, p_drop, seed, y, B, Hh, Ww, C, coef, GROUPS, EPS)
+                return coef
+            if x_parts is not None:
+                H.gn_coef_from_partials(x_parts, B, Hh * Ww, gn.weight, gn.bias, film, coef, GROUPS, EPS)
+            else:
+                stats = self._new(x, B, GROUPS, 2)
+                H.gn_stats(x, _ld(x), B, Hh * Ww, C, stats, GROUPS, EPS)
+            H.gn_apply_v(x, _ld(x), stats, gn.weight, gn.bias, film, act, p_drop, seed, y, B, Hh, Ww, C, coef, GROUPS)
+            return coef
         if x_parts is not None and H.GN_FOLD and max(k for _, _, k in x_parts) <= H.GN_FOLD_MAX_CHUNKS:
             H.gn_apply_from_partials(x, _ld(x), x_parts, gn.weight, gn.bias, film, act, p_drop, seed, rs, y, _ld(y), B, Hh, Ww, C, coef,
                                      GROUPS, EPS)
@@ -229,15 +241,16 @@
         if len(q) == H.GROUP_MAX:
             self._wgrad_flush_key(key)
 
-    def _cwgrad(self, x, ldx, dy, lddy, *args, **kw):
+    def _cwgrad(self, x, ldx, dy, lddy, *args, v=False, **kw):
+        run = (lambda: H.conv3x3_wgrad_wino43_v(x, dy, lddy, *args, **kw)) if v else (lambda: H.conv3x3_wgrad(x, ldx, dy, lddy, *args, **kw))
         side = self._side
         if side is None:
-            return H.conv3x3_wgrad(x, ldx, dy, lddy, *args, **kw)
+            return run()
         side.wait_stream(torch.cuda.current_stream())
         x.record_stream(side)
         dy.record_stream(side)
         with torch.cuda.stream(side):
-            H.conv3x3_wgrad(x, ldx, dy, lddy, *args, **kw)
+            run()
 
     def _side_join(self):
         if self._side is not None:
@@ -359,6 +372,14 @@
         H.conv3x3(x, ldx, self._pack_d(w) if dgrad else self._pack_f(w), bias, y, ldy, B, Hh, Ww, Cin, Cout, res=res, ldres=ldres,
                   stats_part=stats_part)
         return H.last_row_tile() // 2
+
+    def _v_path(self, w, B, Hh, Ww, Cin, Cout, ldy, ldres=0, train=True):
+        return (self._layer(w).u43f is not None and H.v_handover_supported(B, Hh, Ww, Cin, Cout, ldy, ldres)
+                and (not train or H.wgrad43_supported(B, Hh, Ww, Cin, Cout, Cin, Cout)))
+
+    def _conv_v(self, V, w, bias, y, ldy, B, Hh, Ww, Cin, Cout, res=None, ldres=0, stats_part=None):
+        H.conv3x3_wino43_fwd_v(V, self._layer(w).u43f, bias, y, ldy, B, Hh, Ww, Cin, Cout, res=res, ldres=ldres, stats_part=stats_part)
+        return H.wino43_fwd_chunk_rows(Hh, Ww)
 
     def _pack_f(self, w, cin_p=None):
         p = self._layer(w)
@@ -502,16 +523,21 @@
         B, Hh, Ww, Cin, ldx = _chk(x)
         Cout, rs = blk.cout, blk.rs
         Ho, Wo = (Hh // 2, Ww // 2) if rs == H.RS_DOWN else ((Hh * 2, Ww * 2) if rs == H.RS_UP else (Hh, Ww))
-        a1 = self._new(x, B, Ho, Wo, Cin)
-        coef1 = self._norm(x, x_parts, mod.norm1, None, 1, 0.0, 0, rs, a1, B, Hh, Ww, Cin)
+        v1 = rs == H.RS_NONE and self._v_path(mod.conv1.weight, B, Ho, Wo, Cin, Cout, Cout, train=tape is not None)
+        a1 = self._new(x, 36 * B * (Ho // 4) * (Wo // 4) * Cin) if v1 else self._new(x, B, Ho, Wo, Cin)
+        coef1 = self._norm(x, x_parts, mod.norm1, None, 1, 0.0, 0, rs, a1, B, Hh, Ww, Cin, v_out=v1)
         h1 = self._new(x, B, Ho, Wo, Cout)
         ph = self._part(x, B, Ho * Wo, Cout)
-        rows = self._conv(a1, Cin, mod.conv1.weight, mod.conv1.bias, h1, Cout, B, Ho, Wo, Cin, Cout, stats_part=ph)
+        if v1:
+            rows = self._conv_v(a1, mod.conv1.weight, mod.conv1.bias, h1, Cout, B, Ho, Wo, Cin, Cout, stats_part=ph)
+        else:
+            rows = self._conv(a1, Cin, mod.conv1.weight, mod.conv1.bias, h1, Cout, B, Ho, Wo, Cin, Cout, stats_part=ph)
         h1_parts = self._parts(ph, Cout, Ho * Wo, rows)
         c2, fi = self.film_slot[prefix]
         film = films[c2][fi]
-        a2 = self._new(x, B, Ho, Wo, Cout)
-        coef2 = self._norm(h1, h1_parts, mod.norm2, film, 1, p_drop, seed, H.RS_NONE, a2, B, Ho, Wo, Cout)
+        v2 = self._v_path(mod.conv2.weight, B, Ho, Wo, Cout, Cout, _ld(dest), max(ldx, Cout), train=tape is not None)
+        a2 = self._new(x, 36 * B * (Ho // 4) * (Wo // 4) * Cout) if v2 else self._new(x, B, Ho, Wo, Cout)
+        coef2 = self._norm(h1, h1_parts, mod.norm2, film, 1, p_drop, seed, H.RS_NONE, a2, B, Ho, Wo, Cout, v_out=v2)
         if rs != H.RS_NONE:
             xs = self._new(x, B, Ho, Wo, Cin)
             H.gn_apply(x, ldx, None, None, None, None, 0, 0.0, 0, rs, xs, Cin, B, Hh, Ww, Cin, None, GROUPS)
@@ -525,12 +551,16 @@
         else:
             sk = xs
         pd = self._part(x, B, Ho * Wo, Cout)
-        rows = self._conv(a2, Cout, mod.conv2.weight, mod.conv2.bias, dest, _ld(dest), B, Ho, Wo, Cout, Cout, res=sk,
-                          ldres=_ld(sk), stats_part=pd)
+        if v2:
+            rows = self._conv_v(a2, mod.conv2.weight, mod.conv2.bias, dest, _ld(dest), B, Ho, Wo, Cout, Cout, res=sk, ldres=_ld(sk),
+                                stats_part=pd)
+        else:
+            rows = self._conv(a2, Cout, mod.conv2.weight, mod.conv2.bias, dest, _ld(dest), B, Ho, Wo, Cout, Cout, res=sk,
+                              ldres=_ld(sk), stats_part=pd)
         out_parts = self._parts(pd, Cout, Ho * Wo, rows)
         if tape is not None:
             tape[prefix] = dict(x=x, coef1=coef1, a1=a1, h1=h1, coef2=coef2, a2=a2, film=film, xs=xs if has_skip else None,
-                                seed=seed, p=p_drop)
+                                seed=seed, p=p_drop, v1=v1, v2=v2)
         return out_parts
 
     def _res_bwd(self, blk, mod, prefix, ctx, dy, dx, dx_accumulate, ta, dfilms, G):
@@ -539,7 +569,7 @@
         _, Ho, Wo, Cout, lddy = _chk(dy)
         rs = blk.rs
         self._cwgrad(a2, Cout, dy, lddy, B, Ho, Wo, Cout, Cout, G[prefix + ".conv2.weight"], Cout, Cout,
-                        dbias=G[prefix + ".conv2.bias"])
+                        dbias=G[prefix + ".conv2.bias"], v=ctx["v2"])
         da2 = self._new(x, B, Ho, Wo, Cout)
         self._conv(dy, lddy, mod.conv2.weight, None, da2, Cout, B, Ho, Wo, Cout, Cout, dgrad=True)
         dh1 = self._new(x, B, Ho, Wo, Cout)
@@ -550,7 +580,7 @@
                        pgb_keep=self._pgb(B, Cout, G[prefix + ".norm2.weight"], G[prefix + ".norm2.bias"]))
         del da2
         self._cwgrad(a1, Cin, dh1, Cout, B, Ho, Wo, Cin, Cout, G[prefix + ".conv1.weight"], Cin, Cout,
-                        dbias=G[prefix + ".conv1.bias"])
+                        dbias=G[prefix + ".conv1.bias"], v=ctx["v1"])
         da1 = self._new(x, B, Ho, Wo, Cin)
         self._conv(dh1, Cout, mod.conv1.weight, None, da1, Cin, B, Ho, Wo, Cout, Cin, dgrad=True)
         del dh1
```

New measurement: 2132. 1.8% lower.
